# aptx4869lm/4DCapture-FPV

Hardware: AMD Instinct MI355X
Metric: frames/sec global-opt (fixed iters), 1024f clip/500k-pt scene; Chamfer GB/s (higher is better)
Workload: dtype f32; 1 GPU; BASELINE config 3: 1024-frame clip, 500000-pt scene, 500 contact verts, 500 Adam iterations (phase split 0.8), full loss; frames sharded over 1 GPU(s); frames=1024, scene_points=500000, contact_verts=500, iters=500, body_verts=10475, lbs_weights_per_vertex=4

## Files before the change

### 4dcapture-fpv_amd/capi.py

```python
from __future__ import annotations

import ctypes
import os
from ctypes import POINTER, c_char_p, c_double, c_float, c_int32, c_int64, c_void_p

import numpy as np

_HERE = os.path.dirname(os.path.abspath(__file__))
LIB_PATH = os.environ.get("FDCAP_LIB") or os.path.join(_HERE, "libfdcap_hip.so")

NUM_LOSSES = 8
XDIM = 78
PDIM = 75


class FdcapError(RuntimeError):
    pass


class ModelDesc(ctypes.Structure):
    _fields_ = [("num_verts", c_int32), ("v_template", POINTER(c_float)), ("shapedirs", POINTER(c_float)),
                ("num_shape", c_int32), ("posedirs", POINTER(c_float)), ("J_regressor", POINTER(c_float)),
                ("parents", POINTER(c_int32)), ("lbs_weights", POINTER(c_float)),
                ("hands_componentsl", POINTER(c_float)), ("hands_componentsr", POINTER(c_float)),
# ... 29 lines not shown
    "fdcap_debug_scene_hash": (c_int32, [c_void_p, c_void_p]),
    "fdcap_debug_scene_table": (c_int32, [c_void_p, c_int32, c_void_p, POINTER(c_int64)]),
    "fdcap_debug_kernel_forms": (c_int32, [c_void_p, c_int32, c_int32]),
    "fdcap_debug_pose_joint_sets": (c_int32, [c_void_p, c_void_p]),
    "fdcap_set_contact_ids": (c_int32, [c_void_p, c_void_p, c_int32]),
    "fdcap_chamfer_fwd": (c_int32, [c_void_p, c_void_p, c_void_p, c_int32, c_int32, c_int32, c_int64, c_void_p,
                                     c_void_p, c_void_p, c_void_p, c_void_p]),
    "fdcap_chamfer_bwd": (c_int32, [c_void_p, c_void_p, c_void_p, c_int32, c_int32, c_int32, c_int64, c_void_p,
                                     c_void_p, c_void_p, c_void_p]),
    "fdcap_chamfer_fwd_scene": (c_int32, [c_void_p, c_void_p, c_int32, c_int32, c_void_p, c_void_p, c_int32, c_void_p]),
    "fdcap_chamfer_bwd_scene": (c_int32, [c_void_p, c_void_p, c_int32, c_int32, c_void_p, c_void_p, c_void_p, c_void_p]),
    "fdcap_set_nn_kernel": (c_int32, [c_int32]),
    "fdcap_vposer_decode": (c_int32, [c_void_p, c_void_p, c_int32, c_int32, c_void_p, c_void_p, c_void_p]),
    "fdcap_vposer_decode_bwd": (c_int32, [c_void_p, c_void_p, c_int32, c_int32, c_void_p, c_void_p, c_void_p, c_void_p]),
    "fdcap_smplx_backward": (c_int32, [c_void_p] * 7 + [c_int32] + [c_void_p] * 9),
    "fdcap_body_forward": (c_int32, [c_void_p, c_void_p, c_int32, c_void_p, c_void_p, c_void_p]),
    "fdcap_world_mesh": (c_int32, [c_void_p, c_void_p, c_int32, c_void_p, c_void_p, c_void_p, c_void_p]),
    "fdcap_params_75_to_78": (c_int32, [c_void_p, c_int32, c_void_p, c_void_p]),
    "fdcap_params_78_to_75": (c_int32, [c_void_p, c_int32, c_void_p, c_void_p]),
    "fdcap_smplx_forward": (c_int32, [c_void_p, c_void_p, c_void_p, c_void_p, c_void_p, c_void_p, c_void_p, c_int32,
                                       c_void_p, c_void_p, c_void_p]),
    "fdcap_opt_create": (c_int32, [c_void_p, POINTER(OptConfig), c_void_p, c_void_p, c_void_p, c_void_p, c_void_p]),
    "fdcap_opt_create_clips": (c_int32, [c_void_p, POINTER(OptConfig), c_int32, c_void_p, c_void_p, c_void_p, c_void_p, c_void_p]),
    "fdcap_opt_create_clips_var": (c_int32, [c_void_p, POINTER(OptConfig), c_int32, POINTER(c_int32), c_void_p, c_void_p, c_void_p, c_void_p,
                                             c_void_p]),
    "fdcap_opt_set_inputs": (c_int32, [c_void_p, c_void_p, c_void_p, c_void_p, c_void_p, c_void_p]),
    "fdcap_opt_backward": (c_int32, [c_void_p, c_int32, c_int32, c_int32, c_void_p]),
    "fdcap_opt_step": (c_int32, [c_void_p, c_int32, c_int32, c_void_p]),
    "fdcap_opt_backward_and_step": (c_int32, [c_void_p, c_int32, c_int32, c_int32, c_void_p]),
    "fdcap_opt_sync": (c_int32, [c_void_p, c_void_p]),
    "fdcap_opt_run": (c_int32, [c_void_p, c_int32, c_int32, c_int32, c_int32, c_int32, c_void_p, c_int32, c_int32, c_void_p, c_void_p]),
    "fdcap_comm_unique_id": (c_int32, [c_void_p]),
    "fdcap_comm_create": (c_int32, [c_void_p, c_void_p, c_int32, c_int32]),
    "fdcap_comm_destroy": (c_int32, [c_void_p]),
    "fdcap_comm_last_error": (c_char_p, [c_void_p]),
    "fdcap_opt_halo_exchange": (c_int32, [c_void_p, c_void_p]),
    "fdcap_opt_exchange": (c_int32, [c_void_p, c_int32, c_int32, c_void_p]),
    "fdcap_opt_time_exchange": (c_int32, [c_void_p, c_int32, POINTER(c_float), POINTER(c_float), c_void_p]),
    "fdcap_comm_allreduce_f64": (c_int32, [c_void_p, c_void_p, c_int32, c_void_p]),
    "fdcap_opt_state_len": (c_int32, [c_void_p]),
    "fdcap_opt_export_state": (c_int32, [c_void_p, c_void_p, c_void_p]),
    "fdcap_opt_import_state": (c_int32, [c_void_p, c_void_p, c_void_p]),
    "fdcap_opt_check_finite": (c_int32, [c_void_p, c_void_p, c_void_p]),
    "fdcap_opt_set_loss_output": (c_int32, [c_void_p, c_void_p]),
    "fdcap_opt_detect_contact": (c_int32, [c_void_p, c_int32, c_void_p, c_void_p]),
    "fdcap_opt_backward_local2": (c_int32, [c_void_p, c_void_p, c_int32, c_void_p]),
    "fdcap_opt_step_x": (c_int32, [c_void_p, c_int32, c_void_p]),
    "fdcap_opt_set_dct": (c_int32, [c_void_p, c_void_p, c_int32, c_int32, c_void_p, c_void_p]),
    "fdcap_opt_dct_fit": (c_int32, [c_void_p, c_int32, c_int32, c_float, c_void_p, c_int32, c_void_p]),
    "fdcap_opt_backward_dct": (c_int32, [c_void_p, c_float, c_float, c_float, c_int32, c_void_p]),
    "fdcap_opt_set_dct_coef": (c_int32, [c_void_p, c_void_p, c_void_p]),
    "fdcap_opt_get_dct": (c_int32, [c_void_p, c_void_p, c_void_p]),
    "fdcap_opt_get_dct_state": (c_int32, [c_void_p, c_void_p, c_void_p, c_void_p]),
    "fdcap_opt_set_dct_state": (c_int32, [c_void_p, c_void_p, c_void_p, c_void_p]),
    "fdcap_opt_dct_windows": (c_int32, [c_void_p, POINTER(c_int32), POINTER(c_int32)]),
    "fdcap_frame_smoother": (c_int32, [c_void_p, c_void_p, c_int32, c_int32, c_float, c_float, c_float, c_float,
                                        c_void_p, c_int32, c_int32, c_void_p, c_void_p]),
    "fdcap_opt_set_keypoints": (c_int32, [c_void_p, c_void_p, c_void_p]),
    "fdcap_opt_backward_fit2d": (c_int32, [c_void_p, POINTER(Fit2dStage), c_int32, c_void_p]),
    "fdcap_opt_reset_adam": (c_int32, [c_void_p, c_void_p]),
    "fdcap_lbfgs_create": (c_int32, [c_int32, POINTER(LbfgsConfig), POINTER(c_void_p)]),
    "fdcap_lbfgs_destroy": (None, [c_void_p]),
    "fdcap_lbfgs_reset": (c_int32, [c_void_p, c_void_p]),
    "fdcap_lbfgs_advance": (c_int32, [c_void_p, c_void_p, c_int32, c_void_p, c_void_p, c_int32, c_void_p, c_void_p]),
    "fdcap_lbfgs_get_stats": (c_int32, [c_void_p, c_void_p, c_void_p, c_void_p, c_void_p]),
    "fdcap_lbfgs_finalize": (c_int32, [c_void_p, c_void_p, c_int32, c_void_p, c_void_p]),
    "fdcap_opt_fit2d_lbfgs": (c_int32, [c_void_p, POINTER(Fit2dStage), POINTER(LbfgsConfig), c_int32, POINTER(c_int32), c_void_p]),
    "fdcap_opt_fit2d_lbfgs_stats": (c_int32, [c_void_p, c_void_p, c_void_p, c_void_p, c_void_p]),
    "fdcap_opt_step_rows_and_pack": (c_int32, [c_void_p, c_int32, c_int32, c_void_p, c_void_p]),
    "fdcap_opt_unpack_and_step_scale": (c_int32, [c_void_p, c_int32, c_int32, c_void_p, c_int32, c_int32, c_void_p]),
    "fdcap_opt_forward_ahead": (c_int32, [c_void_p, c_int32, c_int32, c_int32, c_void_p]),
    "fdcap_exchange_len": (c_int32, []),
    "fdcap_opt_get_results": (c_int32, [c_void_p, c_void_p, c_void_p, c_void_p, c_void_p]),
    "fdcap_opt_destroy": (None, [c_void_p]),
    "fdcap_opt_forward_world": (c_int32, [c_void_p, c_void_p, c_void_p, c_void_p]),
    "fdcap_opt_get_contact": (c_int32, [c_void_p, c_void_p, c_void_p, c_void_p]),
    "fdcap_opt_get_grads": (c_int32, [c_void_p, c_void_p, c_void_p, c_void_p]),
    "fdcap_panel_gemm": (c_int32, [c_void_p, c_int32, c_int32, c_int32, c_void_p, c_int64, c_int64, c_int32, c_void_p, c_int32,
                                   c_void_p]),
    "fdcap_time_blend_gemm": (c_int32, [c_void_p, c_int32, c_int32, POINTER(c_float), c_void_p]),
    "fdcap_opt_nn_timing": (c_int32, [c_void_p, c_int32]),
    "fdcap_opt_nn_timing_read": (c_int32, [c_void_p, POINTER(c_float), POINTER(c_int32)]),
    "fdcap_debug_nn_query_order": (c_int32, [c_void_p, c_int32, c_void_p, c_int32]),
    "fdcap_debug_nn_query_sort": (c_int32, [c_void_p, c_void_p, c_int32, c_int32, c_int32, c_void_p, c_void_p, c_void_p]),
    "fdcap_opt_launch_timing": (c_int32, [c_void_p, c_int32]),
    "fdcap_opt_launch_timing_read": (c_int32, [c_void_p, c_void_p, c_void_p]),
    "fdcap_opt_time_chamfer": (c_int32, [c_void_p, c_int32, c_int32, POINTER(c_float), c_void_p]),
}

_lib = None


def load_library(path: str | None = None) -> ctypes.CDLL:
    global _lib
    if _lib is not None and path is None:
        return _lib
    p = path or LIB_PATH
    if not os.path.exists(p):
        raise FdcapError(f"{p} is missing: build it with `python -c 'import __graft_entry__ as g; g.build()'` "
                         "(hipcc --offload-arch=gfx950).  There is no CPU fallback.")
    lib = ctypes.CDLL(p)
    for name, (res, args) in SYMBOLS.items():
        fn = getattr(lib, name)
        fn.restype = res
        fn.argtypes = args
    info = lib.fdcap_build_info().decode()
    if "packed_fp32=off" not in info and os.environ.get("FDCAP_ALLOW_PK_F32") != "1":
        raise FdcapError(f"{p} was built with packed fp32 instructions ({info}): results are not reliable next to another kernel's "
                         "MFMAs on the same CU (NOTES.md section 6).  Rebuild with __graft_entry__.build(), or set "
                         "FDCAP_ALLOW_PK_F32=1 for an instrumentation variant.")
    if path is None:
        _lib = lib
    return lib


def count_packed_fp32(path: str | None = None) -> int:
    import re
    import shutil
    import subprocess
    import tempfile
    objdump = os.environ.get("LLVM_OBJDUMP", "/opt/rocm/lib/llvm/bin/llvm-objdump")
    if not os.path.exists(objdump):
        raise FdcapError(f"{objdump} not found (set LLVM_OBJDUMP)")
    with tempfile.TemporaryDirectory() as tmp:
        so = os.path.join(tmp, "lib.so")
        shutil.copy(path or LIB_PATH, so)
        subprocess.run([objdump, "--offloading", so], check=True, capture_output=True, cwd=tmp)
        objs = [f for f in os.listdir(tmp) if "amdgcn" in f]
        if not objs:
            raise FdcapError("no gfx950 code object found in the library")
        n = 0
        for f in objs:
            txt = subprocess.run([objdump, "-d", os.path.join(tmp, f)], check=True, capture_output=True, text=True).stdout
            n += len(re.findall(r"\bv_pk_(?:fma|mul|add)_f32\b", txt))
        return n


def check(code: int, what: str) -> None:
    if code == 0:
        return
    if code < 0:
        names = {-1: "FDCAP_E_ARG", -2: "FDCAP_E_STATE", -3: "FDCAP_E_NODEVICE", -4: "FDCAP_E_COMM (RCCL)"}
        raise FdcapError(f"{what}: {names.get(code, code)}")
    raise FdcapError(f"{what}: hipError_t {code}")


def _f32(a):
    return np.ascontiguousarray(a, dtype=np.float32)


def _fp(a):
    return a.ctypes.data_as(POINTER(c_float))


def dptr(t):
    if t is None:
        return None
    if not t.is_cuda:
        raise FdcapError("expected a device tensor (the HIP path has no host fallback)")
    if not t.is_contiguous():
        raise FdcapError("expected a contiguous tensor")
    return c_void_p(t.data_ptr())


def current_stream():
    import torch
# ... 58 lines not shown
```

### 4dcapture-fpv_amd/csrc/fdc_api_opt.h

```cpp
#pragma once

extern "C" {

void fdcap_opt_destroy(fdcap_ctx* c) {
    if (!c || !c->opt) return;
    OptState* o = c->opt;
    DevBuf<float>* fb[] = {&o->X0, &o->mask, &o->mX, &o->vX, &o->mCAM, &o->vCAM, &o->mS, &o->vS,
                           &o->H1, &o->H2, &o->O, &o->dO, &o->Opart, &o->dZpart, &o->Rm, &o->PF, &o->Jrest, &o->G, &o->A, &o->M,
                           &o->Jw, &o->Voff, &o->Vw, &o->dist, &o->pd, &o->dVoff, &o->dA, &o->dtransl_v, &o->dMv,
                           &o->dsv, &o->dPF, &o->dJw, &o->dX, &o->dCAM, &o->dscale_row, &o->loss_rows, &o->VoffF, &o->VwF, &o->dVF};
    for (auto* b : fb) b->release();
    o->dctD.release(); o->dctCoef.release(); o->dctM.release(); o->dctV.release(); o->adam_tab.release();
    o->clip_rows.release(); o->clip_span.release();
    o->idx.release(); o->pi.release(); o->seedpt.release(); o->kp2d.release(); o->floss.release();
    if (o->lbfgs) { fdcap_lbfgs_destroy(o->lbfgs); o->lbfgs = nullptr; }
    o->nnc_ids.release(); o->nnc_hdr.release(); o->nnc_anchor.release();
    for (hipEvent_t e : o->nn_ev) (void)hipEventDestroy(e);
    o->nn_ev.clear();
    for (hipEvent_t e : o->lt.ev) (void)hipEventDestroy(e);
    o->lt.ev.clear(); o->lt.what.clear(); o->lt.on = false; o->lt.used = 0;
    delete o;
    c->opt = nullptr;
}

static_assert(LROW == FDCAP_NUM_LOSSES, "a batch's per-clip loss slots are LROW apart on the device");
static_assert(CLIP_XDIM == XDIM && CLIP_NJW == NJW, "fdc_clips.h restates the two dimensions its weights divide by");
static_assert(POSE_NJ == NJ && POSE_NJW == NJW, "fdc_forms.h restates the two joint counts plan_pose_joints works with");

static LossWeights opt_phase_weights(const fdcap_opt_config& cf, bool phase2) {
    LossWeights lw;
    lw.rec = 1.f;
    lw.smooth = phase2 ? cf.phase2_smooth : cf.phase1_smooth;
    lw.contact = phase2 ? 0.f : cf.phase1_contact;
    lw.world = phase2 ? cf.phase2_world : 0.f;
    lw.dct = 0.f;
    lw.world_on = phase2;
    return lw;
}

static int opt_create_impl(fdcap_ctx* c, const fdcap_opt_config* cfg, int32_t n_clips, const int32_t* var_len, float* rows_x, float* rows_cam,
                           float* scale_d, float* dscale_d, double* losses_d) {
    SetupTrace tr("fdcap_opt_create");
    OptState* o = c->opt ? c->opt : new OptState();
    c->opt = o;
    o->cfg = *cfg;
    o->nclip = n_clips;
    o->clip_len = var_len ? 0 : cfg->n_total;
    o->ragged = var_len != nullptr;
    if (var_len) o->clip_lens.assign(var_len, var_len + n_clips);
    else o->clip_lens.assign((size_t)n_clips, cfg->n_total);
    o->clip_start = clip_starts(n_clips, o->clip_lens.data());
    if (n_clips > 1 && !var_len) o->cfg.n_total = o->cfg.n_local = n_clips * cfg->n_total;
    cfg = &o->cfg;
    o->cam_steps = 0;
    o->dz_pending = false;
    o->log_pending = false;
    o->seeded = false;
    o->dctT = o->dctC = o->dctW = 0;
    o->dct_grad = false;
    const int R = o->R = cfg->n_local + 4;
    o->contact_on = c->ns > 0 && c->nc > 0 && cfg->weight_contact != 0.f;
    const size_t nq = (size_t)R * std::max(c->nc, 1);
    o->sw = forms_read_env();
    { const char* e = getenv("FDCAP_POSE_TRIM"); o->sw.pose_trim = !(e && e[0] == '0'); }
    const int nq_all = (int)((size_t)cfg->n_local * c->nc);
    o->nsplit = o->contact_on ? nn_pick_nsplit(nq_all, (int)c->ns, o->sw.nn_seed && o->sw.nn_cull) : 1;
    o->nsplit_bf = o->contact_on ? nn_pick_nsplit(nq_all, (int)c->ns, false) : 1;
    int err = 0;
#define AL(buf, cnt) if (!err) { hipError_t e_ = (buf).ensure(cnt); if (e_ != hipSuccess) err = (int)e_; else e_ = hipMemset((buf).p, 0, (size_t)(cnt) * sizeof(*(buf).p)); }
    o->X.p = rows_x; o->CAM.p = rows_cam; o->scale.p = scale_d; o->dscale.p = dscale_d; o->losses.p = losses_d;
    o->pend.on = false;
    AL(o->X0, (size_t)R * XDIM) AL(o->mask, R)
    AL(o->mX, (size_t)R * XDIM) AL(o->vX, (size_t)R * XDIM) AL(o->mCAM, (size_t)R * 16) AL(o->vCAM, (size_t)R * 16)
    AL(o->mS, n_clips) AL(o->vS, n_clips)
    AL(o->H1, (size_t)R * 512) AL(o->H2, (size_t)R * 512) AL(o->O, (size_t)R * O_LD) AL(o->dO, (size_t)R * ODIM)
    AL(o->Opart, (size_t)4 * R * ODIM) AL(o->dZpart, (size_t)4 * R * VP_Z)
    AL(o->Rm, (size_t)R * RM_LD) AL(o->PF, (size_t)R * NPFX) AL(o->Jrest, (size_t)R * JR_LD) AL(o->G, (size_t)R * NJ * 12)
    AL(o->A, (size_t)R * NJ * 12) AL(o->M, (size_t)R * 12) AL(o->Jw, (size_t)R * NJW * 3)
    AL(o->dA, (size_t)R * NJ * 12) AL(o->dtransl_v, (size_t)R * 3) AL(o->dMv, (size_t)R * 12)
    AL(o->dsv, R) AL(o->dPF, (size_t)2 * R * NPFX)
    AL(o->dJw, (size_t)R * NJW * 3) AL(o->dX, (size_t)R * XDIM)
    AL(o->dCAM, (size_t)R * 16) AL(o->dscale_row, R) AL(o->loss_rows, (size_t)R * LROW)
    if (o->contact_on) {
        AL(o->Voff, nq * 3) AL(o->Vw, nq * 3) AL(o->dist, nq) AL(o->idx, nq) AL(o->dVoff, nq * 3) AL(o->seedpt, nq)
        AL(o->pd, (size_t)std::max(o->nsplit, o->nsplit_bf) * nq) AL(o->pi, (size_t)std::max(o->nsplit, o->nsplit_bf) * nq)
    }
#undef AL
    tr.mark("buffers");
    if (!err && o->contact_on) {
        hipError_t e_ = hipMemset(o->idx.p, 0xFF, nq * sizeof(int));
        if (e_ != hipSuccess) err = (int)e_;
    }
    if (!err && o->contact_on) {
        const int every = o->sw.nn_order;
        o->nn_order = NNOrder{};
        if (o->sw.nn_cache_slack > 0.f) {
            const size_t ng = ((size_t)nq_all + 31) / 32, ng4 = ng * 4;
            hipError_t e_ = o->nnc_ids.ensure(ng4 * NN_CACHE_CAP);
            if (e_ == hipSuccess) e_ = o->nnc_hdr.ensure(ng4 + 3 * ng);
            if (e_ == hipSuccess) e_ = o->nnc_anchor.ensure((size_t)4 * nq_all);
            if (e_ == hipSuccess && every > 0) e_ = o->nnq_buf.ensure(nn_query_order_ints(nq_all));
            if (e_ == hipSuccess) e_ = hipMemset(o->nnc_hdr.p, 0xFF, ng4 * sizeof(int));
            if (e_ == hipSuccess) e_ = hipMemset(o->nnc_hdr.p + ng4, 0, 3 * ng * sizeof(int));
            if (e_ == hipSuccess) e_ = hipMemset(o->nnc_anchor.p, 0, (size_t)4 * nq_all * sizeof(float4));
            if (e_ != hipSuccess) err = (int)e_;
            if (every > 0) { o->nn_order.on = true; o->nn_order.every = every; o->nn_order.qbuf = o->nnq_buf.p; }
        }
    }
    if (!err) {
        const std::vector<float> s((size_t)n_clips, cfg->scale_init);
        hipError_t e_ = hipMemcpy(o->scale.p, s.data(), s.size() * sizeof(float), hipMemcpyHostToDevice);
        if (e_ != hipSuccess) err = (int)e_;
    }
    if (!err && o->ragged) {
        std::vector<ClipRow> rows = clip_rows_build(n_clips, var_len, opt_phase_weights(*cfg, false), cfg->weight_loss_rec, cfg->weight_contact, c->nc);
        const std::vector<ClipRow> rows2 = clip_rows_build(n_clips, var_len, opt_phase_weights(*cfg, true), cfg->weight_loss_rec, cfg->weight_contact, c->nc);
        rows.insert(rows.end(), rows2.begin(), rows2.end());
        std::vector<int> span((size_t)2 * n_clips);
        for (int k = 0; k < n_clips; ++k) { span[(size_t)2 * k] = o->clip_start[(size_t)k]; span[(size_t)2 * k + 1] = var_len[k]; }
        hipError_t e_ = rows.size() == (size_t)2 * R ? o->clip_rows.upload(rows.data(), rows.size()) : hipErrorInvalidValue;
        if (e_ == hipSuccess) e_ = o->clip_span.upload(span.data(), span.size());
        if (e_ != hipSuccess) err = (int)e_;
    }
    tr.mark("search state");
    if (err) { fdcap_opt_destroy(c); return err; }
    return FDCAP_OK;
}

int fdcap_opt_create_clips(fdcap_ctx* c, const fdcap_opt_config* cfg, int32_t n_clips, float* rows_x, float* rows_cam, float* scale_d,
                           float* dscale_d, double* losses_d) {
    if (!c || !cfg || !rows_x || !rows_cam || !scale_d || !dscale_d || !losses_d || cfg->n_local <= 0 || cfg->n_total < cfg->n_local || cfg->frame0 < 0 ||
        cfg->frame0 + cfg->n_local > cfg->n_total || n_clips < 1)
        return FDCAP_E_ARG;
    if (n_clips > 1 && (cfg->frame0 != 0 || cfg->n_local != cfg->n_total || (int64_t)n_clips * cfg->n_total > (1 << 24)))
        return FDCAP_E_ARG;
    return opt_create_impl(c, cfg, n_clips, nullptr, rows_x, rows_cam, scale_d, dscale_d, losses_d);
}

int fdcap_opt_create_clips_var(fdcap_ctx* c, const fdcap_opt_config* cfg, int32_t n_clips, const int32_t* clip_len, float* rows_x, float* rows_cam,
                               float* scale_d, float* dscale_d, double* losses_d) {
    if (!c || !cfg || !rows_x || !rows_cam || !scale_d || !dscale_d || !losses_d || cfg->frame0 != 0 || cfg->n_local != cfg->n_total ||
        !clip_lengths_ok(n_clips, clip_len, cfg->n_total, (int64_t)1 << 24))
        return FDCAP_E_ARG;
    if (clip_lengths_equal(n_clips, clip_len)) {
        fdcap_opt_config one = *cfg;
        one.n_total = one.n_local = clip_len[0];
        return fdcap_opt_create_clips(c, &one, n_clips, rows_x, rows_cam, scale_d, dscale_d, losses_d);
// ... 49 lines not shown
    const bool timed = o->nn_timing && o->nn_ev_used + 2 <= (int)o->nn_ev.size();
    if (timed) HIP_TRY(hipEventRecord(o->nn_ev[o->nn_ev_used], st));
    {
        TraceRange tr_("fdcap:chamfer_nn(K14)");
        HIP_TRY(nn_search(o->Vw.p + off, nq, c->nn_target(o->sw.nn_cull), o->dist.p + 2 * nc, o->idx.p + 2 * nc, o->pd.p, o->pi.p,
                          o->nsplit, st, o->sw.nn_seed ? o->idx.p + 2 * nc : nullptr, !o->seeded, o->seedpt.p + 2 * nc, &o->nnpt_valid,
                          &cache, &o->nn_order));
    }
    if (timed) { HIP_TRY(hipEventRecord(o->nn_ev[o->nn_ev_used + 1], st)); o->nn_ev_used += 2; }
    lt_mark(o, FDCAP_LT_CHAMFER_NN, st);
    o->seeded = true;
    return 0;
}

static int opt_backward_impl(fdcap_ctx* c, const LossWeights& lw, int32_t log_terms, hipStream_t st, int fuse_ii = -1, int fuse_P = 0) {
    OptState* o = c->opt;
    const fdcap_opt_config& cf = o->cfg;
    const int nl = cf.n_local, nc = c->nc, N = o->clip_len, rpc = o->rows_per_clip(), kn = o->kclip_n();
    const ClipRow* ctab = nullptr;
    if (o->ragged) {
        const auto same = [&lw](const LossWeights& t) {
            return t.rec == lw.rec && t.smooth == lw.smooth && t.contact == lw.contact && t.world == lw.world && t.dct == lw.dct && t.world_on == lw.world_on;
        };
        if (same(opt_phase_weights(cf, false))) ctab = o->ctab(false);
        else if (same(opt_phase_weights(cf, true))) ctab = o->ctab(true);
        else return FDCAP_E_STATE;
    }
    const int* const cspan = o->cspan();
    const bool dct_on = lw.dct != 0.f && o->dctW > 0;
    PoseModel pm = c->pose_model();
    TraceRange tr_(fuse_ii >= 0 ? "fdcap:backward_and_step" : "fdcap:backward");
    if (o->log_pending) {
        hipLaunchKernelGGL(loss_rows_reduce_kernel, dim3(o->nclip), dim3(256), 0, st, o->loss_rows.p, 2, rpc, o->log_mask, o->log_assign, o->log_dst,
                           o->dscale_row.p, o->dscale.p, cspan);
        o->log_pending = false;
    }
    double* const losses = log_terms ? o->losses.p : nullptr;
    const bool rows_log = losses && o->dctW == 0;
    if (losses && !rows_log) HIP_TRY(hipMemsetAsync(losses, 0, (size_t)o->nclip * FDCAP_NUM_LOSSES * sizeof(double), st));
    int row_lo, row_hi;
    opt_row_range(o, 1, &row_lo, &row_hi);
    const bool ahead = o->ahead, blend_done = o->ahead && o->ahead_blend;
    const bool contact_grad = o->contact_on && lw.contact != 0.f;
    const bool contact_fwd = o->contact_on && (contact_grad || log_terms);
    o->lt.phase = contact_grad ? 0 : 1;
    const bool contact_state = contact_fwd || (dct_on || o->dctW > 0);
    const bool need_world = lw.world_on || dct_on || o->dctW > 0 || log_terms != 0 || ahead || cf.n_local != cf.n_total;
    const PoseJoints pj = plan_pose_joints(c->h_parents.data(), c->h_depth.data(), contact_fwd ? c->contact.ja_hi : 0, contact_state, need_world,
                                           o->sw.pose_trim && o->dctW == 0);
    if (contact_grad && (pj.jr != NJ || pj.jn < c->contact.ja_hi)) return FDCAP_E_STATE;
    int e = ahead ? opt_pose_forward_rest(c, row_lo, row_hi, st) : opt_pose_forward(c, row_lo, row_hi, st, contact_state, &pj);
    o->ahead = false;
    if (e) return e;
    if (contact_fwd) { e = opt_contact_forward(c, st, blend_done); if (e) return e; }
    const ClipWeights cw = clip_weights(std::max(N, 1), lw, cf.weight_loss_rec, cf.weight_contact, nc);
    const float w_rec = cw.w_rec, w_sm = cw.w_sm, w_ws = cw.w_ws;
    const bool fuse_pl = (!losses || rows_log) && !(o->dctW > 0 && dct_on);
    ParamLossIn pli = {};
    if (fuse_pl) pli = ParamLossIn{o->X0.p, o->mask.p, o->Jw.p, cf.frame0, N, w_rec, w_sm, w_ws, lw.world_on ? 1 : 0,
                                   rows_log ? o->loss_rows.p : nullptr};
    else if (ctab) return FDCAP_E_STATE;
    else
        hipLaunchKernelGGL(param_loss_kernel, dim3(nl), dim3(128), 0, st, o->X.p, o->X0.p, o->mask.p, o->Jw.p, 2, cf.frame0, N,
                           w_rec, w_sm, w_ws, lw.world_on ? 1 : 0, o->dX.p, o->dJw.p, losses, kn);
    if (o->dctW > 0 && (dct_on || log_terms))
        hipLaunchKernelGGL(dct_joint_grad_kernel, dim3((nl * 69 + 255) / 256), dim3(256), 0, st, o->Jw.p, 2, cf.frame0, nl, o->dctT,
                           o->dctC, o->dctW, o->dctD.p, o->dctCoef.p, dct_on ? lw.dct / (69.f * (float)o->dctW) : 0.f,
                           lw.world_on ? 1 : 0, o->dJw.p, losses ? losses + 7 : nullptr);
    o->dct_grad = dct_on;
    bool dpf_split = false;
    int dA_rows = NJ;
    if (contact_grad) {
        ContactGradIn cg;
        cg.Vw = o->Vw.p; cg.dist = o->dist.p; cg.idx = o->idx.p; cg.scene = c->scene.p;
        cg.nnpt = o->nnpt_valid ? o->seedpt.p : nullptr;
        cg.coef = cw.coef;
        cg.loss_rows = losses ? o->loss_rows.p : nullptr;
        const SkinModel smc = c->contact.model();
        const int nnz = c->contact.nnz;
        const bool aligned16 = (((size_t)o->Vw.p | (size_t)o->Voff.p | (size_t)o->dVoff.p | (size_t)o->A.p) & 15) == 0;
        const SkinBwdPlan pl = plan_contact_skin_bwd(nl, nc, nnz, smc.K, smc.vpack != nullptr, smc.csc_v16 != nullptr, aligned16, smc.wf_tab != nullptr,
                                                     o->sw.skin_vec);
        if (pl.ja_rows) dA_rows = c->contact.ja_hi;
        const dim3 grid(pl.grid), block(pl.block);
#define FDC_SKC(KERNEL) hipLaunchKernelGGL(KERNEL, grid, block, pl.lds, st, smc, nc, nnz, o->X.p, o->Voff.p, o->A.p, o->M.p, o->scale.p, 2, o->dVoff.p, \
                                           o->dA.p, o->dtransl_v.p, o->dMv.p, o->dsv.p, cg, kn, ctab)
        switch (pl.form) {
        case F_SKIN_BWD_VEC:
            note_form(form_name(pl.form));
            if (pl.G == 1) FDC_SKC(skin_bwd_vec_kernel<1>); else if (pl.G == 2) FDC_SKC(skin_bwd_vec_kernel<2>); else FDC_SKC(skin_bwd_vec_kernel<3>);
            break;
        case F_SKIN_BWD_SMALL: case F_SKIN_BWD_SMALL_K:
            note_form(form_name(pl.form));
            if (pl.vpt == 2 && pl.kc == 8) FDC_SKC((skin_bwd_small_kernel<2, 8>));
            else if (pl.vpt == 2) FDC_SKC((skin_bwd_small_kernel<2, 24>));
            else if (pl.kc == 16) FDC_SKC((skin_bwd_small_kernel<4, 16>));
            else FDC_SKC((skin_bwd_small_kernel<4, 24>));
            break;
        default:
            { int es = skin_bwd_any<true>(c->ws_skin, st, nl, smc, nc, o->X.p, o->Voff.p, o->A.p, o->M.p, o->scale.p, 2,
                                          (const float*)nullptr, o->dVoff.p, o->dA.p, (float*)nullptr, o->dtransl_v.p, o->dMv.p, o->dsv.p, cg, kn, ctab);
              if (es) return es; }
        }
#undef FDC_SKC
        lt_mark(o, FDCAP_LT_SKIN_BWD, st);
        HIP_TRY(blend_backward(c->contact, o->dVoff.p + (size_t)2 * nc * 3, nl, o->dPF.p + 2 * NPFX, (size_t)o->R * NPFX, c->ws_kpart, st, &dpf_split));
        lt_mark(o, FDCAP_LT_BLEND_BWD, st);
    } else if (contact_fwd && losses) {
        if (fuse_pl && rows_log) { pli.cdist = o->dist.p; pli.cnc = nc; }
        else hipLaunchKernelGGL(contact_loss_rows_kernel, dim3(nl), dim3(256), 0, st, o->dist.p, nc, 2, o->loss_rows.p);
    }
    const bool joint_grad = lw.world_on || dct_on;
    hipLaunchKernelGGL(pose_bwd_kernel, dim3(nl), dim3(64 * POSE_NW), 0, st, pm, o->X.p, o->O.p, o->CAM.p, o->scale.p, 2, o->Rm.p,
                       o->Jrest.p, o->G.p, contact_grad ? o->dA.p : nullptr, contact_grad ? o->dPF.p : nullptr,
                       joint_grad ? o->dJw.p : nullptr, contact_grad ? o->dMv.p : nullptr, contact_grad ? o->dsv.p : nullptr,
                       contact_grad ? o->dPF.p + NPF : nullptr, NPFX, contact_grad ? o->dtransl_v.p : nullptr, o->dX.p, o->dO.p,
                       o->dCAM.p, o->dscale_row.p, pli, (contact_grad && dpf_split) ? (const float*)(o->dPF.p + (size_t)o->R * NPFX) : (const float*)nullptr,
                       dA_rows, kn, ctab, pj.jn, pj.jr, pj.nlev);
    o->pj_bwd = pj;
    lt_mark(o, FDCAP_LT_POSE_BWD, st);
    const unsigned log_mask = (rows_log ? 0x17u : 0u) | (contact_fwd ? 0x8u : 0u);
    bool log_in_tail = false;
    {
        ScaleTail tail;
        if (fuse_ii >= 0) {
            const StepPlan sp = opt_step_plan(o, fuse_ii, fuse_P, false, true);
            tail.dscale_row = o->dscale_row.p; tail.row0 = 2;
            if (sp.step_scale) {
                tail.block = 0; tail.sc = sp.sc; tail.dscale = o->dscale.p; tail.n = rpc;
                tail.zero_grad = fuse_ii >= fuse_P ? 1 : 0;
            }
            if (log_terms == 2 && rows_log) {
                tail.block = 0; tail.lg = LogReduceIn{o->loss_rows.p, losses, log_mask, 1, rpc};
                log_in_tail = true;
            }
        }
        int eb = opt_vposer_backward(c, false, st, tail);
        if (eb) return eb;
        if (fuse_ii >= 0) { o->pend.on = true; o->pend.ii = fuse_ii; o->pend.P = fuse_P; }
    }
    if (log_terms && !log_in_tail) {
        if (log_terms == 2 && rows_log) {
            o->log_pending = true; o->log_mask = log_mask; o->log_assign = 1; o->log_dst = losses;
        } else
            hipLaunchKernelGGL(loss_rows_reduce_kernel, dim3(o->nclip), dim3(256), 0, st, o->loss_rows.p, 2, rpc, log_mask, rows_log ? 1 : 0, losses,
                               o->dscale_row.p, o->dscale.p, cspan);
    }
    return (int)hipGetLastError();
}

int fdcap_opt_set_loss_output(fdcap_ctx* c, double* losses_d) {
    if (!c || !c->opt || !losses_d) return FDCAP_E_ARG;
    c->opt->log_pending = false;
    c->opt->log_dst = nullptr;
    c->opt->losses.p = losses_d;
    return FDCAP_OK;
}

int fdcap_opt_forward_ahead(fdcap_ctx* c, int32_t ii, int32_t P, int32_t log_terms, void* stream) {
    if (!c || !c->opt || c->opt->nclip > 1) return FDCAP_E_STATE;
    { int es_ = opt_sync(c, (hipStream_t)stream); if (es_) return es_; }
    OptState* o = c->opt;
    hipStream_t st = (hipStream_t)stream;
    const int nl = o->cfg.n_local, nc = c->nc;
    int e = opt_pose_forward(c, 2, 2 + nl, st);
    if (e) return e;
// ... 78 lines not shown
```

### 4dcapture-fpv_amd/csrc/fdc_api_run.h

```cpp
#pragma once

extern "C" {

int fdcap_opt_detect_contact(fdcap_ctx* c, int32_t n_left, float* weight_left, void* stream) {
    if (opt_is_batch(c)) return FDCAP_E_STATE;
    if (!c || !c->opt || !weight_left || n_left <= 0 || n_left > c->nc) return FDCAP_E_ARG;
    OptState* o = c->opt;
    if (!o->contact_on) return FDCAP_E_STATE;
    hipStream_t st = (hipStream_t)stream;
    const int nl = o->cfg.n_local, nc = c->nc;
    int row_lo, row_hi;
    opt_row_range(o, 1, &row_lo, &row_hi);
    int e = opt_pose_forward(c, row_lo, row_hi, st);
    if (e) return e;
    e = opt_contact_forward(c, st);
    if (e) return e;
    hipLaunchKernelGGL(detect_contact_kernel, dim3(nl), dim3(256), 0, st, o->dist.p, c->contact_perm.p, nc, n_left, 2, weight_left);
    return (int)hipGetLastError();
}

int fdcap_opt_backward_local2(fdcap_ctx* c, const float* contact_weight, int32_t n_left, void* stream) {
    if (opt_is_batch(c)) return FDCAP_E_STATE;
    if (!c || !c->opt || !contact_weight || n_left <= 0 || n_left >= c->nc) return FDCAP_E_ARG;
    { int es_ = opt_sync(c, (hipStream_t)stream); if (es_) return es_; }
// ... 200 lines not shown
    int e = comm_buffers(c);
    if (e) return e;
    hipEvent_t ev[4];
    for (auto& x : ev) HIP_TRY(hipEventCreate(&x));
    const int big = 1 << 30;
    for (int k = 0; k < 8 && !e; ++k) e = fdcap_opt_exchange(c, k, big, stream);
    if (!e) e = (int)hipEventRecord(ev[0], st);
    for (int k = 0; k < iters && !e; ++k) e = fdcap_opt_exchange(c, 8 + k, big, stream);
    if (!e) e = (int)hipEventRecord(ev[1], st);
    if (!e) e = (int)hipEventRecord(ev[2], st);
    for (int k = 0; k < iters && !e; ++k) {
        const ncclResult_t r = rccl().AllGather(c->xch_send.p, c->xch_all.p, XCH_LEN, ncclFloat, c->comm.comm, st);
        if (r != ncclSuccess) e = comm_fail(c, r, "ncclAllGather");
    }
    if (!e) e = (int)hipEventRecord(ev[3], st);
    if (!e) e = (int)hipEventSynchronize(ev[3]);
    float a = 0.f, b = 0.f;
    if (!e) e = (int)hipEventElapsedTime(&a, ev[0], ev[1]);
    if (!e) e = (int)hipEventElapsedTime(&b, ev[2], ev[3]);
    for (auto& x : ev) (void)hipEventDestroy(x);
    *us_exchange = a * 1e3f / iters;
    *us_allgather = b * 1e3f / iters;
    return e;
}

int fdcap_opt_run(fdcap_ctx* c, int32_t ii0, int32_t ii1, int32_t num_iter, int32_t P, int32_t log_every, double* hist_d,
                  int32_t hist_rows, int32_t flags, int32_t* n_logged, void* stream) {
    if (n_logged) *n_logged = 0;
    if (!c || !c->opt) return FDCAP_E_STATE;
    if (ii0 < 0 || ii1 < ii0 || ii1 > num_iter || log_every < 0) return FDCAP_E_ARG;
    OptState* o = c->opt;
    const bool sharded = (flags & 2) != 0 || !opt_whole_clips(o);
    if (sharded && (!c->comm.comm || o->nclip > 1)) return FDCAP_E_STATE;
    const size_t hist_row = (size_t)o->nclip * FDCAP_NUM_LOSSES;
    double* const keep = o->losses.p;
    int k = 0, e = 0;
    for (int ii = ii0; ii < ii1 && !e; ++ii) {
        const bool do_log = log_every > 0 && (ii % log_every == 0 || ii == num_iter - 1);
        if (do_log) {
            if (!hist_d || k >= hist_rows) { e = FDCAP_E_ARG; break; }
            e = fdcap_opt_set_loss_output(c, hist_d + (size_t)k * hist_row);
            if (e) break;
            ++k;
        }
        const int lt = do_log ? 2 : 0;
        if (sharded) {
            e = fdcap_opt_backward(c, ii, P, lt, stream);
            if (!e) e = fdcap_opt_exchange(c, ii, P, stream);
        } else if (!(flags & 1) && ii + 1 < num_iter) {
            e = fdcap_opt_backward_and_step(c, ii, P, lt, stream);
        } else {
            e = fdcap_opt_backward(c, ii, P, lt, stream);
            if (!e) e = fdcap_opt_step(c, ii, P, stream);
        }
    }
    if (k) {
        const int e2 = fdcap_opt_set_loss_output(c, keep);
        if (!e) e = e2;
    }
    if (n_logged) *n_logged = k;
    return e;
}

int fdcap_comm_allreduce_f64(fdcap_ctx* c, double* buf_d, int32_t n, void* stream) {
    if (!c || !buf_d || n <= 0) return FDCAP_E_ARG;
    if (!c->comm.comm) return FDCAP_E_STATE;
    const ncclResult_t r = rccl().AllReduce(buf_d, buf_d, (size_t)n, ncclDouble, ncclSum, c->comm.comm, (hipStream_t)stream);
    if (r != ncclSuccess) return comm_fail(c, r, "ncclAllReduce");
    return FDCAP_OK;
}

int fdcap_opt_get_contact(fdcap_ctx* c, float* dist, int32_t* idx, void* stream) {
    if (!c || !c->opt) return FDCAP_E_STATE;
    OptState* o = c->opt;
    if (!o->contact_on) return FDCAP_E_STATE;
    hipStream_t st = (hipStream_t)stream;
    const size_t n = (size_t)o->cfg.n_local * c->nc;
    const int nl = o->cfg.n_local, nc = c->nc;
    if (dist) hipLaunchKernelGGL(unpermute_kernel<float>, dim3((n + 255) / 256), dim3(256), 0, st, o->dist.p + 2 * nc,
                                 c->contact_perm.p, nl, nc, 1, dist);
    if (idx) hipLaunchKernelGGL(unpermute_kernel<int>, dim3((n + 255) / 256), dim3(256), 0, st, o->idx.p + 2 * nc,
                                c->contact_perm.p, nl, nc, 1, idx);
    return (int)hipGetLastError();
}

int fdcap_opt_get_grads(fdcap_ctx* c, float* dx, float* dcam, void* stream) {
    if (!c || !c->opt) return FDCAP_E_STATE;
    { int es_ = opt_sync(c, (hipStream_t)stream); if (es_) return es_; }
    OptState* o = c->opt;
    hipStream_t st = (hipStream_t)stream;
    const int nl = o->cfg.n_local;
    if (o->dz_pending) {
        hipLaunchKernelGGL(vposer_fold_dz_kernel, dim3((nl * VP_Z + 255) / 256), dim3(256), 0, st, o->dZpart.p, (size_t)o->R * VP_Z, 2, nl, o->dX.p);
        o->dz_pending = false;
    }
    if (dx) HIP_TRY(hipMemcpyAsync(dx, o->dX.p + 2 * XDIM, (size_t)nl * XDIM * sizeof(float), hipMemcpyDeviceToDevice, st));
    if (dcam) HIP_TRY(hipMemcpyAsync(dcam, o->dCAM.p + 2 * 16, (size_t)nl * 16 * sizeof(float), hipMemcpyDeviceToDevice, st));
    return FDCAP_OK;
}

int fdcap_panel_gemm(const float* A, int32_t lda, int32_t M, int32_t K, const float* B_h, int64_t sk, int64_t sn, int32_t N, float* C,
                     int32_t ldc, void* stream) {
    if (!A || !B_h || !C || M <= 0 || K <= 0 || N <= 0 || lda < K || ldc < N) return FDCAP_E_ARG;
    hipStream_t st = (hipStream_t)stream;
    {
        if (forms_read_env().gemm_split3 && panel_gemm3_fits(K)) {
            std::vector<unsigned> p3;
            std::vector<float> sc;
            PanelB3 B3;
            PnF::pack(B_h, (long)sk, (long)sn, K, N, p3, sc, &B3.ntile, &B3.nst);
            DevBuf<unsigned> d3;
            DevBuf<float> ds;
            HIP_TRY(d3.upload(p3.data(), p3.size()));
            HIP_TRY(ds.upload(sc.data(), sc.size()));
            B3.f = (const uint4*)d3.p; B3.isc = ds.p;
            hipError_t e = panel_gemm3(A, lda, M, K, B3, C, ldc, N, st);
            hipError_t e2 = hipStreamSynchronize(st);
            d3.release(); ds.release();
            return (int)(e != hipSuccess ? e : e2);
        }
    }
    std::vector<float> pf;
    PanelB B;
    panel_pack(B_h, (long)sk, (long)sn, K, N, pf, &B.ntile, &B.nss);
    DevBuf<float> d;
    HIP_TRY(d.upload(pf.data(), pf.size()));
    B.f = (const float4*)d.p;
    hipError_t e = panel_gemm(A, lda, M, K, B, C, ldc, N, st);
    hipError_t e2 = hipStreamSynchronize(st);
    d.release();
    return (int)(e != hipSuccess ? e : e2);
}

int fdcap_opt_nn_timing(fdcap_ctx* c, int32_t max_launches) {
    if (!c || !c->opt || max_launches < 0) return FDCAP_E_ARG;
    OptState* o = c->opt;
    o->nn_timing = max_launches > 0;
    o->nn_ev_used = 0;
    while ((int)o->nn_ev.size() < 2 * max_launches) {
        hipEvent_t e;
        HIP_TRY(hipEventCreate(&e));
        o->nn_ev.push_back(e);
    }
    return FDCAP_OK;
}
int fdcap_opt_nn_timing_read(fdcap_ctx* c, float* mean_ms, int32_t* launches) {
    if (!c || !c->opt || !mean_ms || !launches) return FDCAP_E_ARG;
    OptState* o = c->opt;
    double sum = 0.0;
    for (int i = 0; i + 1 < o->nn_ev_used; i += 2) {
        HIP_TRY(hipEventSynchronize(o->nn_ev[i + 1]));
        float t = 0.f;
        HIP_TRY(hipEventElapsedTime(&t, o->nn_ev[i], o->nn_ev[i + 1]));
        sum += t;
    }
    *launches = o->nn_ev_used / 2;
    *mean_ms = *launches ? (float)(sum / *launches) : 0.f;
    return FDCAP_OK;
}

int fdcap_opt_launch_timing(fdcap_ctx* c, int32_t max_events) {
    if (!c || !c->opt || max_events < 0) return FDCAP_E_ARG;
    OptState::LaunchTimes& t = c->opt->lt;
    t.on = max_events > 0;
    t.used = 0;
    while ((int)t.ev.size() < max_events) {
// ... 95 lines not shown
```

### 4dcapture-fpv_amd/csrc/fdc_chamfer.h

```cpp
#pragma once
#include <hip/hip_runtime.h>
#include <stdlib.h>

#include <atomic>

#include "fdc_forms.h"
#include "fdc_math.h"

namespace fdc {

constexpr int NN_TILE = 1024;

struct NNTarget {
    const float4* pts;
    int n;
    const float4* bounds;
    const float4* sbounds;
    const float4* qbounds;
    const int* inv_perm;
    const uint4* frags;
    const float4* centers;
};

__device__ __forceinline__ float nn_exact_d2(float qx, float qy, float qz, float px, float py, float pz) {
    float dx = qx - px, dy = qy - py, dz = qz - pz;
    return __fmaf_rn(dz, dz, __fmaf_rn(dy, dy, __fmul_rn(dx, dx)));
}
__device__ __forceinline__ bool nn_better(float d, int i, float bd, int bi) {
    return d < bd || (d == bd && i < bi);
}

__device__ __forceinline__ void nn_block_map(int b, int nsplit, int* qb, int* split) {
    const int xcd = b & 7, slot = b >> 3;
    *split = slot % nsplit;
    *qb = (slot / nsplit) * 8 + xcd;
}

template <int QPT>
__global__ __launch_bounds__(256) void nn_direct_kernel(const float* __restrict__ q, int nq, NNTarget T, int nsplit,
                                                        float* __restrict__ pd, int* __restrict__ pi) {
    __shared__ float4 tile[NN_TILE];
    const int tid = threadIdx.x;
    int split, qb;
    nn_block_map(blockIdx.x, nsplit, &qb, &split);
    if (qb * (256 * QPT) >= nq) return;
    const int per = nn_split_len(T.n, nsplit);
    const int t_begin = min(T.n, split * per);
    const int t_end = min(T.n, t_begin + per);
    float qx[QPT], qy[QPT], qz[QPT], best[QPT];
    int bi[QPT];
#pragma unroll
    for (int u = 0; u < QPT; ++u) {
        int qi = qb * (256 * QPT) + u * 256 + tid;
        bool ok = qi < nq;
        qx[u] = ok ? q[3 * (size_t)qi] : 0.f;
        qy[u] = ok ? q[3 * (size_t)qi + 1] : 0.f;
        qz[u] = ok ? q[3 * (size_t)qi + 2] : 0.f;
        best[u] = INFINITY;
        bi[u] = -1;
    }
    for (int base = t_begin; base < t_end; base += NN_TILE) {
        const int cnt = min(NN_TILE, t_end - base);
        for (int j = tid; j < cnt; j += 256) tile[j] = T.pts[base + j];
        __syncthreads();
#pragma unroll 4
        for (int j = 0; j < cnt; ++j) {
            const float4 p = tile[j];
            const int gi = __float_as_int(p.w);
#pragma unroll
            for (int u = 0; u < QPT; ++u) {
                float d = nn_exact_d2(qx[u], qy[u], qz[u], p.x, p.y, p.z);
                if (nn_better(d, gi, best[u], bi[u])) { best[u] = d; bi[u] = gi; }
            }
        }
        __syncthreads();
    }
#pragma unroll
    for (int u = 0; u < QPT; ++u) {
        int qi = qb * (256 * QPT) + u * 256 + tid;
        if (qi < nq) {
            pd[(size_t)split * nq + qi] = best[u];
            pi[(size_t)split * nq + qi] = bi[u];
        }
    }
}

#ifndef FDC_MF_K1
#define FDC_MF_K1 1e-4f
#endif
#ifndef FDC_MF_K2
#define FDC_MF_K2 8e-6f
#endif
constexpr float MF_K1 = FDC_MF_K1, MF_K2 = FDC_MF_K2;

#ifdef FDC_NN_TIMELINE
__device__ unsigned long long g_nn_timeline[16384 * 8];
#endif
#ifdef FDC_NN_STATS
__device__ unsigned long long g_nn_hist[96];
__device__ unsigned long long g_nn_stats[8];
#define FDC_STAT(i, v) st_cnt[i] += (v)
#else
#define FDC_STAT(i, v)
#endif

typedef __bf16 bf16x8 __attribute__((ext_vector_type(8)));
typedef float f32x16_t __attribute__((ext_vector_type(16)));

__device__ __forceinline__ unsigned f2bf(float f) {
    __bf16 h = (__bf16)f;
    return (unsigned)__builtin_bit_cast(unsigned short, h);
}
__device__ __forceinline__ float bf2f(unsigned h) { return __uint_as_float(h << 16); }
// ... 201 lines not shown
                    FDC_STAT(1, lane == 0);
#pragma unroll
                    for (int r = 0; r < 16; ++r) {
                        if (acc[r] < thr[n]) {
                            FDC_STAT(2, 1);
                            const int row = (r & 3) + 8 * (r >> 2) + 4 * half;
                            const float4 p = sP[buf][tile * 32 + row];
                            const int gi = __float_as_int(p.w);
                            const float d = nn_exact_d2(qx[n], qy[n], qz[n], p.x, p.y, p.z);
                            if (base + tile * 32 + row < t_end && nn_better(d, gi, own_d[n], own_i[n])) {
                                own_d[n] = d;
                                own_i[n] = gi;
                                thr[n] = mf_thr(d, X[n], X2[n]);
                            }
                        }
                    }
                    const float sb = fminf(own_d[n], __shfl_xor(own_d[n], 32, 64));
                    if (qidx[n] < nq) thr[n] = mf_thr(sb, X[n], X2[n]);
                }
            }
        }
        if (more) stage_write(buf ^ 1, nxt);
        __syncthreads();
        buf ^= 1;
    }
#ifdef FDC_NN_STATS
    for (int i = 0; i < 8; ++i) atomicAdd(&g_nn_stats[i], (unsigned long long)st_cnt[i]);
#endif
#pragma unroll
    for (int n = 0; n < NQ; ++n) {
        float od = __shfl_xor(own_d[n], 32, 64);
        int oi = __shfl_xor(own_i[n], 32, 64);
        if (oi >= 0 && (own_i[n] < 0 || nn_better(od, oi, own_d[n], own_i[n]))) { own_d[n] = od; own_i[n] = oi; }
        if (half == 0 && qidx[n] < nq) {
            pd[(size_t)split * nq + qidx[n]] = own_d[n];
            pi[(size_t)split * nq + qidx[n]] = own_i[n];
        }
    }
}


#ifndef FDC_ST4_MAXLIST
#define FDC_ST4_MAXLIST 768
#endif
#ifndef FDC_ST4_MAXCELL
#define FDC_ST4_MAXCELL 256
#endif
constexpr int ST4_MAXLIST = FDC_ST4_MAXLIST;
constexpr int ST4_MAXCELL = FDC_ST4_MAXCELL;
#ifndef FDC_ST4_PF
#define FDC_ST4_PF 2
#endif
#ifndef FDC_AS_MULT
#define FDC_AS_MULT 4.f
#endif
#ifndef FDC_AS_MAX
#define FDC_AS_MAX 3.f
#endif
#ifndef FDC_AS_NEAR
#define FDC_AS_NEAR 0.8f
#endif
#ifndef FDC_ST4_OCC
#define FDC_ST4_OCC 8
#endif
#ifndef FDC_ST4_OCC2
#define FDC_ST4_OCC2 3
#endif
constexpr int ST4_PF = FDC_ST4_PF;
constexpr int ST4_SUPER = 16;
constexpr int ST4_QCAP = 8;

#ifndef FDC_NN_CACHE_CAP
#define FDC_NN_CACHE_CAP 128
#endif
constexpr int NN_CACHE_CAP = FDC_NN_CACHE_CAP;
static_assert(NN_CACHE_CAP == 64 || NN_CACHE_CAP == 128, "one or two ids per lane");
struct NNCache {
    unsigned short* ids;
    int* hdr;
    float4* anchor;
    float slack;
    int order_mode = 0;
    const int* perm = nullptr;
};

template <int NQ, int WPG, int WPB = 4>
__global__ __launch_bounds__(64 * WPB, NQ == 1 ? FDC_ST4_OCC : FDC_ST4_OCC2) void nn_stream4_kernel(const float* __restrict__ q, int nq, NNTarget T,
                                                         const int* __restrict__ seed, float4* __restrict__ seedpt,
                                                         float* __restrict__ dist, int* __restrict__ idx, NNCache cache) {
    __shared__ unsigned short slist[WPB][ST4_MAXLIST];
    __shared__ unsigned short clist[WPB][ST4_MAXCELL];
    __shared__ float4 sbox[WPB][64][2];
    __shared__ float s_d[WPB][32 * NQ];
    __shared__ int s_i[WPB][32 * NQ];
    __shared__ float4 s_p[WPB][32 * NQ];
    __shared__ int s_q[WPB][32 * NQ];
    static_assert(WPG == 1 || WPG == 2 || WPG == 4, "waves per query group");
    static_assert(WPB % WPG == 0 && WPB <= 4, "a group's waves share a workgroup");
    constexpr int GPW = WPB / WPG;
    constexpr int CPS = ST4_SUPER / WPG;
    const int tid = threadIdx.x, wave = tid >> 6, lane = tid & 63, half = lane >> 5, col = lane & 31;
    const int sub = wave % WPG, gslot = wave / WPG;
    const int ngroups = (nq + 32 * NQ - 1) / (32 * NQ);
    const int nwg = (ngroups + GPW - 1) / GPW;
#ifdef FDC_NN_TIMELINE
    const unsigned long long tl_t0 = wall_clock64();
    unsigned long long tl_p[4] = {0, 0, 0, 0};
#define TL_STAMP(k) tl_p[k] = wall_clock64()
#else
#define TL_STAMP(k)
#endif
    const int wg = (cache.order_mode >= 2 && (int)blockIdx.x < nwg) ? cache.hdr[(3 + cache.order_mode) * ((nq + 31) / 32) + (int)blockIdx.x] : (int)blockIdx.x;
    const int group = wg * GPW + gslot;
    const bool idle = wg >= nwg || group >= ngroups;
    const int wq0 = idle ? nq : group * (32 * NQ);
    const int nchunk = (T.n + MF_CH - 1) / MF_CH;
    const int myn = idle ? 0 : (nchunk - sub + WPG - 1) / WPG;
#ifdef FDC_NN_STATS
    unsigned st_cnt[8] = {0, 0, 0, 0, 0, 0, 0, 0};
#endif
    const bool caching = cache.hdr != nullptr && !idle;
    const int cidx = group * WPG + sub;
    float lqx[NQ], lqy[NQ], lqz[NQ];
    int lsj[NQ];
    float4 lsp[NQ];
    const int* const perm = NQ == 1 && WPB == 1 ? cache.perm : nullptr;
#pragma unroll
    for (int n = 0; n < NQ; ++n) {
        size_t qc = (size_t)min(wq0 + n * 32 + col, nq - 1);
        if (perm) {
            qc = (size_t)perm[qc];
            if (half == 0) s_q[wave][n * 32 + col] = (int)qc;
        }
        lqx[n] = q[3 * qc]; lqy[n] = q[3 * qc + 1]; lqz[n] = q[3 * qc + 2];
        lsj[n] = seed[qc];
        lsp[n] = seedpt[qc];
    }
    int hv_pre = -1;
    unsigned id_pre = 0;
    float4 anc_pre[NQ];
#pragma unroll
    for (int n = 0; n < NQ; ++n) anc_pre[n] = make_float4(0.f, 0.f, 0.f, -1.f);
    if (caching) {
        hv_pre = cache.hdr[cidx];
        id_pre = NN_CACHE_CAP == 64 ? (unsigned)cache.ids[(size_t)cidx * NN_CACHE_CAP + lane]
                                    : ((const unsigned*)cache.ids)[(size_t)cidx * (NN_CACHE_CAP / 2) + lane];
#pragma unroll
        for (int n = 0; n < NQ; ++n) anc_pre[n] = cache.anchor[(size_t)sub * nq + min(wq0 + n * 32 + col, nq - 1)];
    }
#if defined(__HIP_DEVICE_COMPILE__)
#pragma unroll
    for (int n = 0; n < NQ; ++n)
        asm volatile("" : "+v"(lqx[n]), "+v"(lqy[n]), "+v"(lqz[n]), "+v"(lsj[n]), "+v"(lsp[n].x), "+v"(lsp[n].y), "+v"(lsp[n].z), "+v"(lsp[n].w),
                          "+v"(anc_pre[n].x), "+v"(anc_pre[n].y), "+v"(anc_pre[n].z), "+v"(anc_pre[n].w), "+v"(hv_pre), "+v"(id_pre));
#endif
    float qx[NQ], qy[NQ], qz[NQ], own_d[NQ], sb[NQ];
    int own_i[NQ], qidx[NQ];
    float4 own_p[NQ];
    bool all_seeded = true;
#pragma unroll
    for (int n = 0; n < NQ; ++n) {
        qidx[n] = wq0 + n * 32 + col;
        const bool ok = qidx[n] < nq;
        qx[n] = ok ? lqx[n] : 0.f;
        qy[n] = ok ? lqy[n] : 0.f;
        qz[n] = ok ? lqz[n] : 0.f;
        own_d[n] = INFINITY;
        own_i[n] = -1;
        own_p[n] = make_float4(0.f, 0.f, 0.f, __int_as_float(-1));
        const int sj = ok ? lsj[n] : -1;
        const float4 p = ok ? lsp[n] : make_float4(0.f, 0.f, 0.f, 0.f);
        if (ok) {
            if (sj >= 0 && sj < T.n) {
                own_p[n] = p;
                own_d[n] = nn_exact_d2(qx[n], qy[n], qz[n], p.x, p.y, p.z);
                own_i[n] = sj;
            } else {
                all_seeded = false;
            }
        }
        sb[n] = ok ? own_d[n] * 1.00002f + 1e-9f : -INFINITY;
    }
    float rq[NQ];
    bool finite = true;
#pragma unroll
    for (int n = 0; n < NQ; ++n) {
        rq[n] = 0.f;
        if (qidx[n] < nq) {
            rq[n] = __builtin_amdgcn_sqrtf(sb[n]) * 1.00001f + 1e-6f;
            finite &= rq[n] < INFINITY;
        }
    }
    const bool cull = __all(all_seeded && finite);
    TL_STAMP(0);
    auto min_rows01 = [](float v) {
        v = fminf(v, dpp_move<0xB1>(v)); v = fminf(v, dpp_move<0x4E>(v)); v = fminf(v, dpp_move<0x141>(v)); v = fminf(v, dpp_move<0x140>(v));
        return fminf(__int_as_float(__builtin_amdgcn_readlane(__float_as_int(v), 0)), __int_as_float(__builtin_amdgcn_readlane(__float_as_int(v), 16)));
    };
    auto max_rows01 = [](float v) {
        v = fmaxf(v, dpp_move<0xB1>(v)); v = fmaxf(v, dpp_move<0x4E>(v)); v = fmaxf(v, dpp_move<0x141>(v)); v = fmaxf(v, dpp_move<0x140>(v));
        return fmaxf(__int_as_float(__builtin_amdgcn_readlane(__float_as_int(v), 0)), __int_as_float(__builtin_amdgcn_readlane(__float_as_int(v), 16)));
    };

    int n_kept = -1;
    bool inflate = false;
    int slk = __builtin_amdgcn_readfirstlane(__float_as_int(cache.slack));
    if (cull && caching) {
        const int hv = __builtin_amdgcn_readfirstlane(hv_pre);
        bool ok = true;
        float dmax = 0.f;
#pragma unroll
        for (int n = 0; n < NQ; ++n)
            if (qidx[n] < nq) {
                const float4 a = anc_pre[n];
                const float ex = qx[n] - a.x, ey = qy[n] - a.y, ez = qz[n] - a.z;
                const float dl = __builtin_amdgcn_sqrtf(ez * ez + (ey * ey + ex * ex)) * 1.00001f + 1e-7f;
                ok &= rq[n] + dl <= a.w;
                dmax = fmaxf(dmax, dl);
            }
        if (hv >= 0 && __all(ok)) {
            n_kept = hv & 255;
            if (lane == 0) cache.hdr[cidx] = hv + 256;
        } else {
            dmax = max_rows01(dmax);
            dmax = fmaxf(dmax, __shfl_xor(dmax, 32, 64));
            const float age = hv >= 0 ? (float)max(hv >> 8, 1) : 1.f;
            const float speed = dmax / age;
            slk = __builtin_amdgcn_readfirstlane(__float_as_int(fminf(fmaxf(FDC_AS_MULT * speed, cache.slack), FDC_AS_MAX * cache.slack)));
            float smin = __int_as_float(slk);
#pragma unroll
            for (int n = 0; n < NQ; ++n)
                if (qidx[n] < nq && rq[n] > FDC_AS_NEAR) smin = fminf(smin, fmaxf(cache.slack, __int_as_float(slk) * (FDC_AS_NEAR / rq[n])));
            smin = -max_rows01(-smin);
            smin = fminf(smin, __shfl_xor(smin, 32, 64));
            inflate = 3.f * speed <= smin;
        }
    }
    auto slack_of = [&](float r) -> float {
        const float sw = __int_as_float(slk);
        return r <= FDC_AS_NEAR ? sw : fmaxf(cache.slack, sw * (FDC_AS_NEAR / r));
    };
    float sbT[NQ];
    float glx = INFINITY, gly = INFINITY, glz = INFINITY, ghx = -INFINITY, ghy = -INFINITY, ghz = -INFINITY;
    float scx = 0.f, scy = 0.f, scz = 0.f, sR2 = 0.f;
    if (cull && n_kept < 0) {
        float rT[NQ];
#pragma unroll
        for (int n = 0; n < NQ; ++n) {
            rT[n] = inflate ? rq[n] + slack_of(rq[n]) : rq[n];
            sbT[n] = (qidx[n] < nq) ? (inflate ? rT[n] * rT[n] * 1.00002f : sb[n]) : -INFINITY;
        }
#pragma unroll
        for (int n = 0; n < NQ; ++n)
            if (qidx[n] < nq) {
                const float r = rT[n];
                glx = fminf(glx, qx[n] - r); gly = fminf(gly, qy[n] - r); glz = fminf(glz, qz[n] - r);
                ghx = fmaxf(ghx, qx[n] + r); ghy = fmaxf(ghy, qy[n] + r); ghz = fmaxf(ghz, qz[n] + r);
            }
        glx = min_rows01(glx); gly = min_rows01(gly); glz = min_rows01(glz);
        ghx = max_rows01(ghx); ghy = max_rows01(ghy); ghz = max_rows01(ghz);
        scx = 0.5f * (glx + ghx); scy = 0.5f * (gly + ghy); scz = 0.5f * (glz + ghz);
        float sR = 0.f;
#pragma unroll
        for (int n = 0; n < NQ; ++n)
            if (qidx[n] < nq) {
                const float ex = qx[n] - scx, ey = qy[n] - scy, ez = qz[n] - scz;
                sR = fmaxf(sR, (__builtin_amdgcn_sqrtf(ex * ex + ey * ey + ez * ez) + rT[n]) * 1.00001f + 1e-6f);
            }
        sR = max_rows01(sR);
        sR2 = sR * sR * 1.00001f;
    } else {
#pragma unroll
        for (int n = 0; n < NQ; ++n) sbT[n] = sb[n];
    }
    auto overlaps = [&](float4 lo, float4 hi) -> bool {
        return !((lo.x > ghx) | (hi.x < glx) | (lo.y > ghy) | (hi.y < gly) | (lo.z > ghz) | (hi.z < glz)) & (box_d2(lo, hi, scx, scy, scz) <= sR2);
    };
// ... 240 lines not shown
                            unsigned hi = 0;
#pragma unroll
                            for (int r = 15; r >= 9; --r) hi = __builtin_amdgcn_alignbit(hi, __float_as_uint(acc[r] - th), 31);
                            mask |= hi << 9;
                        }
                        if constexpr (NQ == 1) {
                            mask &= (seed_tile == (base >> 5) + tile) ? seed_keep : ~0u;
                        } else {
                            const int spos = __float_as_int(own_p[n].w);
                            const bool mine = (spos >> 5) == (base >> 5) + tile && ((spos >> 2) & 1) == half;
                            if (mine) mask &= ~(1u << ((spos & 3) + 4 * ((spos >> 3) & 3)));
                        }
                        if (!__any(mask != 0)) continue;
                        if constexpr (NQ == 1) {
                            while (mask) {
                                const int r = __ffs(mask) - 1;
                                mask &= mask - 1;
                                const int pos = base + tile * 32 + (r & 3) + 8 * (r >> 2) + 4 * half;
                                if (pos < T.n) {
                                    FDC_STAT(2, 1);
                                    if (cq_n < ST4_QCAP) { cq[cq_n * 64 + lane] = (unsigned)pos; ++cq_n; }
                                    else {
                                        const float4 p = T.pts[pos];
                                        const int gi = __float_as_int(p.w);
                                        const float d = nn_exact_d2(qx[n], qy[n], qz[n], p.x, p.y, p.z);
                                        if (nn_better(d, gi, own_d[n], own_i[n])) {
                                            own_d[n] = d; own_i[n] = gi;
                                            own_p[n] = make_float4(p.x, p.y, p.z, __int_as_float(pos));
                                            seed_refresh();
                                        }
                                    }
                                }
                            }
                            continue;
                        }
                        while (mask) {
                            const int r = __ffs(mask) - 1;
                            mask &= mask - 1;
                            const int pos = base + tile * 32 + (r & 3) + 8 * (r >> 2) + 4 * half;
                            if (pos < T.n && pos != __float_as_int(own_p[n].w)) {
                                FDC_STAT(2, 1);
                                const float4 p = T.pts[pos];
                                const int gi = __float_as_int(p.w);
                                const float d = nn_exact_d2(qx[n], qy[n], qz[n], p.x, p.y, p.z);
                                if (nn_better(d, gi, own_d[n], own_i[n])) {
                                    own_d[n] = d; own_i[n] = gi;
                                    own_p[n] = make_float4(p.x, p.y, p.z, __int_as_float(pos));
                                }
                            }
                        }
                        const float sbest = fminf(own_d[n], __shfl_xor(own_d[n], 32, 64));
                        if (qidx[n] < nq) thr[n] = fminf(thr[n], sbest + c2[n]);
                    }
                }
            }
            ch = ch_next;
            qd = id_next & 3;
            fo = fo_next;
        }
    }
    if constexpr (NQ == 1) {
        for (int k0 = 0; __any(k0 < cq_n); k0 += 4) {
            float4 p[4];
            int ps[4];
#pragma unroll
            for (int k = 0; k < 4; ++k) {
                ps[k] = (k0 + k < cq_n) ? (int)cq[(k0 + k) * 64 + lane] : 0;
                p[k] = T.pts[ps[k]];
            }
#pragma unroll
            for (int k = 0; k < 4; ++k)
                if (k0 + k < cq_n) {
                    const int gi = __float_as_int(p[k].w);
                    const float d = nn_exact_d2(qx[0], qy[0], qz[0], p[k].x, p[k].y, p[k].z);
                    if (nn_better(d, gi, own_d[0], own_i[0])) {
                        own_d[0] = d; own_i[0] = gi;
                        own_p[0] = make_float4(p[k].x, p[k].y, p[k].z, __int_as_float(ps[k]));
                    }
                }
        }
    }
    TL_STAMP(3);
    if (cache.order_mode != 0 && lane == 0 && !idle) cache.hdr[4 * ((nq + 31) / 32) + (int)blockIdx.x] = nsurv;
#pragma unroll
    for (int n = 0; n < NQ; ++n) {
        const float od = __shfl_xor(own_d[n], 32, 64);
        const int oi = __shfl_xor(own_i[n], 32, 64);
        float4 op;
        op.x = __shfl_xor(own_p[n].x, 32, 64); op.y = __shfl_xor(own_p[n].y, 32, 64);
        op.z = __shfl_xor(own_p[n].z, 32, 64); op.w = __shfl_xor(own_p[n].w, 32, 64);
        if (oi >= 0 && (own_i[n] < 0 || nn_better(od, oi, own_d[n], own_i[n]))) { own_d[n] = od; own_i[n] = oi; own_p[n] = op; }
        if (half == 0) { s_d[wave][n * 32 + col] = own_d[n]; s_i[wave][n * 32 + col] = own_i[n]; s_p[wave][n * 32 + col] = own_p[n]; }
    }
    __syncthreads();
#ifdef FDC_NN_STATS
    {
        unsigned mx = st_cnt[2];
        for (int off = 32; off > 0; off >>= 1) mx = max(mx, (unsigned)__shfl_xor((int)mx, off, 64));
        if (lane == 0 && !idle) {
            atomicAdd(&g_nn_hist[32 + (st_cnt[1] > 0 ? 32 - __clz(st_cnt[1]) : 0)], 1ull);
            atomicAdd(&g_nn_hist[64 + (mx > 0 ? 32 - __clz(mx) : 0)], 1ull);
        }
    }
    for (int i = 0; i < 8; ++i) atomicAdd(&g_nn_stats[i], (unsigned long long)st_cnt[i]);
#endif
#ifdef FDC_NN_TIMELINE
    if (tid == 0 && blockIdx.x < 16384) {
        unsigned xcc; asm volatile("s_getreg_b32 %0, hwreg(HW_REG_XCC_ID)" : "=s"(xcc));
        unsigned long long* tl = g_nn_timeline + (size_t)blockIdx.x * 8;
        tl[0] = tl_t0; tl[1] = wall_clock64(); tl[2] = xcc & 15; tl[3] = tl_p[0]; tl[4] = tl_p[1]; tl[5] = tl_p[2]; tl[6] = tl_p[3]; tl[7] = (unsigned long long)tl_nsurv;
    }
#endif
    if (tid < GPW * 32 * NQ) {
        const int g = tid / (32 * NQ), e = tid % (32 * NQ);
        const int qo = (wg * GPW + g) * (32 * NQ) + e;
        if (wg < nwg && qo < nq) {
            int bw = g * WPG;
            float bd = s_d[bw][e];
            int bi = s_i[bw][e];
#pragma unroll
            for (int w = 1; w < WPG; ++w) {
                const float d = s_d[g * WPG + w][e];
                const int i = s_i[g * WPG + w][e];
                if (i >= 0 && (bi < 0 || nn_better(d, i, bd, bi))) { bd = d; bi = i; bw = g * WPG + w; }
            }
            const int qd = perm ? s_q[g][e] : qo;
            dist[qd] = bd;
            idx[qd] = bi;
            seedpt[qd] = s_p[bw][e];
        }
    }
}

__global__ __launch_bounds__(256) void nn_seed_kernel(const float* __restrict__ q, int nq, NNTarget T, int* __restrict__ seed,
                                                      float4* __restrict__ seedpt) {
    const int qi = blockIdx.x * 256 + threadIdx.x;
    if (qi >= nq) return;
    const int old = seed[qi];
    if (old >= 0 && old < T.n) {
        const int pos = T.inv_perm ? T.inv_perm[old] : old;
        const float4 pt = T.pts[pos];
        seedpt[qi] = make_float4(pt.x, pt.y, pt.z, __int_as_float(pos));
        return;
    }
    const float x = q[3 * (size_t)qi], y = q[3 * (size_t)qi + 1], z = q[3 * (size_t)qi + 2];
    const int nchunk = (T.n + MF_CH - 1) / MF_CH;
    float bb = INFINITY;
    int bc = -1;
    int p0, p1;
    if (T.sbounds) {
        const int nsuper = (nchunk + ST4_SUPER - 1) / ST4_SUPER;
        for (int s = 0; s < nsuper; ++s) {
            const float ds = box_d2(T.sbounds[2 * s], T.sbounds[2 * s + 1], x, y, z);
            if (!(ds < bb)) continue;
            for (int c = s * ST4_SUPER; c < min(nchunk, (s + 1) * ST4_SUPER); ++c) {
                const float d = box_d2(T.bounds[2 * c], T.bounds[2 * c + 1], x, y, z);
                if (d < bb) { bb = d; bc = c; }
            }
        }
    } else {
        for (int c = 0; c < nchunk; ++c) {
            const float d = box_d2(T.bounds[2 * c], T.bounds[2 * c + 1], x, y, z);
            if (d < bb) { bb = d; bc = c; }
        }
    }
    if (bc < 0) return;
    float bd = INFINITY;
    int bi = -1;
    float4 bp = make_float4(0.f, 0.f, 0.f, __int_as_float(-1));
    auto scan = [&](int c) {
        p0 = c * MF_CH;
        p1 = min(T.n, p0 + MF_CH);
        for (int p = p0; p < p1; ++p) {
            const float4 pt = T.pts[p];
            const float d = nn_exact_d2(x, y, z, pt.x, pt.y, pt.z);
            if (d < bd) { bd = d; bi = __float_as_int(pt.w); bp = make_float4(pt.x, pt.y, pt.z, __int_as_float(p)); }
        }
    };
    scan(bc);
    if (T.centers) {
        float bm = INFINITY;
        int bc2 = -1;
        auto centre = [&](int c) {
            const float4 cc = T.centers[c];
            const float dx = x - cc.x, dy = y - cc.y, dz = z - cc.z;
            const float m = __builtin_amdgcn_sqrtf(fmaf(dz, dz, fmaf(dy, dy, dx * dx))) + cc.w;
            if (m < bm) { bm = m; bc2 = c; }
        };
        if (T.sbounds) {
            const int nsuper = (nchunk + ST4_SUPER - 1) / ST4_SUPER;
            for (int sb = 0; sb < nsuper; ++sb) {
                if (!(box_d2(T.sbounds[2 * sb], T.sbounds[2 * sb + 1], x, y, z) < bm * bm)) continue;
                for (int c = sb * ST4_SUPER; c < min(nchunk, (sb + 1) * ST4_SUPER); ++c) centre(c);
            }
        } else
            for (int c = 0; c < nchunk; ++c) centre(c);
        if (bc2 >= 0 && bc2 != bc && bm * bm < bd) scan(bc2);
    }
    seed[qi] = bi;
    seedpt[qi] = bp;
}

__global__ void nn_combine_kernel(const float* __restrict__ pd, const int* __restrict__ pi, int nsplit, int nq,
                                  float* __restrict__ dist, int* __restrict__ idx) {
    int qi = blockIdx.x * blockDim.x + threadIdx.x;
    if (qi >= nq) return;
    float best = INFINITY;
    int bi = -1;
    for (int s = 0; s < nsplit; ++s) {
        float d = pd[(size_t)s * nq + qi];
        int j = pi[(size_t)s * nq + qi];
        if (j >= 0 && (bi < 0 || nn_better(d, j, best, bi))) { best = d; bi = j; }
    }
    dist[qi] = best;
    idx[qi] = bi;
}

__global__ void pack_points_kernel(const float* __restrict__ xyz, int n, float4* __restrict__ out) {
    int i = blockIdx.x * blockDim.x + threadIdx.x;
    if (i >= n) return;
    out[i] = make_float4(xyz[3 * (size_t)i], xyz[3 * (size_t)i + 1], xyz[3 * (size_t)i + 2], __int_as_float(i));
}

__global__ void nn_grad_kernel(const float* __restrict__ q, const float4* __restrict__ tgt, const float* __restrict__ g,
                               const int* __restrict__ idx, int nq, float* __restrict__ gq) {
    int qi = blockIdx.x * blockDim.x + threadIdx.x;
    if (qi >= nq) return;
    int j = idx[qi];
    float gg = 2.f * g[qi];
    float4 p = j >= 0 ? tgt[j] : make_float4(0, 0, 0, 0);
    gq[3 * (size_t)qi] = j >= 0 ? gg * (q[3 * (size_t)qi] - p.x) : 0.f;
    gq[3 * (size_t)qi + 1] = j >= 0 ? gg * (q[3 * (size_t)qi + 1] - p.y) : 0.f;
    gq[3 * (size_t)qi + 2] = j >= 0 ? gg * (q[3 * (size_t)qi + 2] - p.z) : 0.f;
}

inline std::atomic<int>& nn_mode_ref() {
    static std::atomic<int> mode{0};
    return mode;
}

__global__ __launch_bounds__(1024) void nn_order_kernel(const int* __restrict__ work, int n, const int* __restrict__ prev,
                                                        int* __restrict__ order) {
    __shared__ int cnt[16][256], base[256];
    const int tid = threadIdx.x, w = tid >> 6;
    for (int e = tid; e < 16 * 256; e += 1024) (&cnt[0][0])[e] = 0;
    __syncthreads();
    for (int i = tid; i < n; i += 1024) atomicAdd(&cnt[w][255 - min(max(work[i], 0), 255)], 1);
    __syncthreads();
    if (tid < 256) {
        int run = 0;
        for (int k = 0; k < 16; ++k) { const int t = cnt[k][tid]; cnt[k][tid] = run; run += t; }
        base[tid] = run;
    }
    __syncthreads();
    if (tid < 64) {
        const int a = base[4 * tid], b = base[4 * tid + 1], c = base[4 * tid + 2], d = base[4 * tid + 3];
        int s = a + b + c + d, incl = s;
        for (int off = 1; off < 64; off <<= 1) { const int t = __shfl_up(incl, off, 64); if (tid >= off) incl += t; }
        const int ex = incl - s;
        base[4 * tid] = ex; base[4 * tid + 1] = ex + a; base[4 * tid + 2] = ex + a + b; base[4 * tid + 3] = ex + a + b + c;
    }
    __syncthreads();
    for (int i = tid; i < n; i += 1024) {
        const int k = 255 - min(max(work[i], 0), 255);
        order[base[k] + atomicAdd(&cnt[w][k], 1)] = prev ? prev[i] : i;
    }
}
struct NNOrder {
    bool on = false;
    int sorted_groups = 0;
    int cur = 0;
    int age = 0;
    int every = 32;
    int* qbuf = nullptr;
    int perm_n = 0;
    int perm_mode = 0;
};
static inline size_t nn_query_order_ints(int nq);
static inline hipError_t nn_query_order(const float4* seedpt, int nq, int* qbuf, int* hdr, int groups, hipStream_t st);

static inline hipError_t nn_search(const float* q, int nq, const NNTarget& T, float* dist, int* idx, float* pd, int* pi,
                                   int nsplit, hipStream_t st, const int* seed = nullptr, bool seed_missing = false,
                                   float4* seedpt = nullptr, bool* seedpt_written = nullptr, const NNCache* cache = nullptr,
                                   NNOrder* ord = nullptr) {
    if (seedpt_written) *seedpt_written = false;
    if (nq <= 0) return hipSuccess;
    const NNPlan pl = plan_nn_search(nq, T.n, seed != nullptr && T.bounds != nullptr, T.frags != nullptr, seedpt != nullptr && seed == idx, nsplit,
                                     nn_mode_ref(), proc_switches());
    const dim3 grid(pl.grid), block(pl.block);
    note_form(form_name(pl.form));
    if (pl.wpg) {
        if (seed_missing)
            hipLaunchKernelGGL(nn_seed_kernel, dim3((nq + 255) / 256), dim3(256), 0, st, q, nq, T, idx, seedpt);
        if (seedpt_written) *seedpt_written = true;
        {
            const int groups = pl.groups, wpg = pl.wpg;
            NNCache nc = cache ? *cache : NNCache{nullptr, nullptr, nullptr, 0.f};
            const bool ordered = ord != nullptr && ord->on && nc.hdr != nullptr && ord->every > 0 && wpg == 1;
            nc.order_mode = !ordered ? 0 : (ord->sorted_groups == groups ? 2 + ord->cur : 1);
            const bool qorder = ordered && ord->qbuf != nullptr && ord->perm_mode != 1;
            nc.perm = qorder && ord->perm_n == nq ? ord->qbuf : nullptr;
            if (wpg == 4) hipLaunchKernelGGL((nn_stream4_kernel<1, 4>), grid, block, 0, st, q, nq, T, seed, seedpt, dist, idx, nc);
            else if (wpg == 2) hipLaunchKernelGGL((nn_stream4_kernel<1, 2>), grid, block, 0, st, q, nq, T, seed, seedpt, dist, idx, nc);
            else hipLaunchKernelGGL((nn_stream4_kernel<1, 1, 1>), grid, block, 0, st, q, nq, T, seed, seedpt, dist, idx, nc);
            const bool resort = ordered && (ord->sorted_groups != groups || ++ord->age >= ord->every);
            if (qorder && ord->perm_mode == 0 && (ord->perm_n != nq || seed_missing || (resort && ord->sorted_groups == groups))) {
                const hipError_t e = nn_query_order(seedpt, nq, ord->qbuf, nc.hdr, groups, st);
                if (e != hipSuccess) return e;
                ord->perm_n = nq;
                ord->sorted_groups = 0;
                ord->age = 0;
            } else if (resort) {
                const bool had = nc.order_mode >= 2;
                const int nxt = had ? 1 - ord->cur : 0;
                hipLaunchKernelGGL(nn_order_kernel, dim3(1), dim3(1024), 0, st, (const int*)(nc.hdr + 4 * groups), groups,
                                   had ? (const int*)(nc.hdr + (5 + ord->cur) * groups) : (const int*)nullptr, nc.hdr + (5 + nxt) * groups);
                ord->cur = nxt;
                ord->sorted_groups = groups;
                ord->age = 0;
            }
        }
        return hipGetLastError();
    }
    if (pl.form == F_NN_MFMA && pl.nq_blocks == 2) hipLaunchKernelGGL((nn_mfma_kernel<2>), grid, block, 0, st, q, nq, T, nsplit, seed, pd, pi);
    else if (pl.form == F_NN_MFMA) hipLaunchKernelGGL((nn_mfma_kernel<4>), grid, block, 0, st, q, nq, T, nsplit, seed, pd, pi);
    else hipLaunchKernelGGL((nn_direct_kernel<2>), grid, block, 0, st, q, nq, T, nsplit, pd, pi);
    hipLaunchKernelGGL(nn_combine_kernel, dim3((nq + 255) / 256), dim3(256), 0, st, pd, pi, nsplit, nq, dist, idx);
    return hipGetLastError();
}

}
```

### 4dcapture-fpv_amd/csrc/fdc_forms.h

```cpp
#pragma once
#include <stddef.h>
#include <stdlib.h>

#include <algorithm>

#if defined(__HIPCC__)
#define FDC_FORMS_HD __host__ __device__
#else
#define FDC_FORMS_HD
#endif

namespace fdc {

struct FormSwitches {
    int clip_fwd_rows = 336;
    int clip_kgrad_rows = 257;
    int pn_rb2 = 1;
    int pn_nw = 0;
    bool pn_ksw = true;
    bool gemm_split3 = true;
    int nn_stream = -2;
    bool nn_seed = true, nn_cull = true;
    int nn_order = 32;
    float nn_cache_slack = 0.03f;
    bool skin_vec = true;
    bool fuse_skin = true;
    bool pose_trim = true;
};
inline FormSwitches forms_read_env() {
    FormSwitches s;
    const auto off = [](const char* name) { const char* e = getenv(name); return e && e[0] == '0'; };
    if (const char* e = getenv("FDCAP_CLIP_FORMS_MIN_ROWS")) s.clip_fwd_rows = s.clip_kgrad_rows = std::max(32, atoi(e));
    if (const char* e = getenv("FDCAP_PN_RB2")) s.pn_rb2 = atoi(e);
    if (const char* e = getenv("FDCAP_PN_NW")) s.pn_nw = atoi(e);
    s.pn_ksw = !off("FDCAP_PN_KSW");
    s.gemm_split3 = !off("FDCAP_GEMM_SPLIT3");
    if (const char* e = getenv("FDCAP_NN_STREAM")) s.nn_stream = atoi(e);
    s.nn_seed = !off("FDCAP_NN_SEED");
    s.nn_cull = !off("FDCAP_NN_CULL");
    if (const char* e = getenv("FDCAP_NN_ORDER")) s.nn_order = atoi(e);
    if (const char* e = getenv("FDCAP_NN_CACHE_SLACK")) s.nn_cache_slack = (float)atof(e);
    s.skin_vec = !off("FDCAP_SKIN_VEC");
    s.fuse_skin = !off("FDCAP_FUSE_SKIN");
    return s;
}
inline const FormSwitches& proc_switches() { static const FormSwitches s = forms_read_env(); return s; }

enum Form {
    F_NONE = 0,
    F_PANEL3, F_PANEL3_RB2, F_PANEL3_WIDE, F_PANEL3_RB2K, F_PANEL3_KSW, F_PANEL3_KLOOP,
    F_BLEND_SKIN_FWD, F_SKIN_FWD,
    F_SKIN_BWD_VEC, F_SKIN_BWD_SMALL, F_SKIN_BWD_SMALL_K, F_SKIN_BWD_FRAME, F_SKIN_BWD_CHUNKS_MFMA, F_SKIN_BWD_CHUNKS_LIST,
    F_NN_STREAM_W4, F_NN_STREAM_W2, F_NN_STREAM_W1, F_NN_MFMA, F_NN_DIRECT,
    F_VPOSER_SPLIT, F_VPOSER_FP32,
    F_COUNT
};
inline const char* form_name(Form f) {
    static const char* const names[F_COUNT] = {
        nullptr,
        "panel_gemm3_kernel", "panel_gemm3_rb2_kernel", "panel_gemm3_wide_kernel", "panel_gemm3_rb2k_kernel", "panel_gemm3_ksw_kernel",
        "panel_gemm3_kloop_kernel",
        "blend_skin_fwd_kernel", "skin_fwd_kernel",
        "skin_bwd_vec_kernel", "skin_bwd_small_kernel", "skin_bwd_small_kernel(K > 4)", "skin_bwd_kernel(one workgroup per frame)",
        "skin_bwd_kernel(chunks, MFMA dA)", "skin_bwd_kernel(chunks, list dA)",
        "nn_stream4_kernel(4 waves per group)", "nn_stream4_kernel(2 waves per group)", "nn_stream4_kernel<1,1,1>", "nn_mfma_kernel",
        "nn_direct_kernel",
        nullptr, nullptr,
    };
    return names[f];
}


constexpr int PN_SC_U4 = 4 + 4 * 12;
constexpr FDC_FORMS_HD int pn_img_u4(int np, int kpad) { return np * (kpad >> 3) * 16 + PN_SC_U4; }
constexpr FDC_FORMS_HD size_t pn_lds_bytes(int np, int kpad, int rb) { return (size_t)rb * pn_img_u4(np, kpad) * 16; }
constexpr int PN3_MAX_K = 2528;
static_assert(pn_lds_bytes(2, PN3_MAX_K, 1) <= 160 * 1024, "one image per CU");
constexpr bool panel_gemm3_fits(int K) { return ((K + 31) & ~31) <= PN3_MAX_K; }
constexpr size_t pn_b_bytes(int np, int ntile, int nst) { return (size_t)ntile * nst * np * 1024; }

struct PnMap { int nrb, ncb, xc, rpg, cpg, rfast; };
inline PnMap panel_map(int nrb, int ncb, size_t a_bytes, size_t b_bytes) {
    PnMap best{nrb, ncb, 1, (nrb + 7) / 8, ncb, 0};
    double best_cost = 1e300;
    for (int xc = 1; xc <= 8; xc *= 2) {
        const int xr = 8 / xc;
        const int rpg = (nrb + xr - 1) / xr, cpg = (ncb + xc - 1) / xc;
        double cost = (double)xc * a_bytes + ((b_bytes / xc <= (size_t)(3u << 19)) ? 0.0 : (double)xr * b_bytes);
        cost *= (double)(8 * rpg * cpg) / (double)(nrb * ncb);
        if (cost < best_cost) { best_cost = cost; best = PnMap{nrb, ncb, xc, rpg, cpg, 0}; }
    }
    best.rfast = b_bytes / best.xc > (size_t)(3u << 19);
    return best;
}

constexpr int PN3_KLOOP_SLAB = 24;
constexpr int PN3_KLOOP_RB = 2, PN3_KLOOP_T = 2;
inline int panel_gemm3_kloop_parts(int M, int ntile) {
    constexpr int rb = PN3_KLOOP_RB, T = PN3_KLOOP_T, wgs = 256;
    const int ncb = (ntile + 8 * T - 1) / (8 * T), nrp = (M + 16 * rb - 1) / (16 * rb);
    int ks = std::min(64, std::max(1, wgs / (ncb * nrp)));
    while (ks > 1 && (ks * ncb) % 8 != 0) --ks;
    if ((ks * ncb) % 8 != 0) { ks = 1; while ((ks * ncb) % 8 != 0 && ks < 64) ++ks; }
    return std::min(ks, 64);
}

struct PanelPlan {
    Form form = F_NONE;
    int nw = 0, T = 0, cs = 0, ks = 0;
    int grid = 0, block = 0;
// ... 193 lines not shown
```

### 4dcapture-fpv_amd/csrc/fdc_k_skin.h

```cpp
#pragma once

namespace {

__global__ __launch_bounds__(256) void skin_fwd_kernel(SkinModel sm, int nv, const float* __restrict__ X, int ldx, int beta_off, int transl_off,
                                const float* __restrict__ Voff, const float* __restrict__ A,
                                const float* __restrict__ M, const float* __restrict__ scale, int row0, int world,
                                float* __restrict__ Vout, int clip_n = 0, const ClipRow* __restrict__ ctab = nullptr) {
    __shared__ __attribute__((aligned(16))) float sA[NJ * 12];
    const int c = blockIdx.x * 256 + threadIdx.x, cc = min(c, nv - 1);
    const int r = row0 + blockIdx.y;
    glds_wg<1, 4, 16>(A + (size_t)r * NJ * 12, sA, NJ * 3);
    const float* x = X + (size_t)r * ldx;
    const V3 transl = v3(x[transl_off], x[transl_off + 1], x[transl_off + 2]);
    float Mr[12] = {1, 0, 0, 0, 0, 1, 0, 0, 0, 0, 1, 0};
    if (world) {
#pragma unroll
        for (int e = 0; e < 12; ++e) Mr[e] = M[(size_t)r * 12 + e];
    }
    const float sc_v = world ? scale[clip_of_row(r, clip_n, ctab)] : 1.f;
    float* o = Vout + ((size_t)r * nv + c) * 3;
    if (sm.vpack && !FDC_SKIN_HAS_S(sm)) {
        const float4* const vp4 = (const float4*)sm.vpack;
        const int G = (sm.K + 3) >> 2;
        const float4 p0 = vp4[cc], p1 = vp4[nv + cc];
        float4 p2 = make_float4(0.f, 0.f, 0.f, 0.f), p3 = p2, pj = p2;
        if (G >= 2) { p2 = vp4[(size_t)2 * nv + cc]; pj = vp4[(size_t)(G + 1) * nv + cc]; }
        if (G >= 3) p3 = vp4[(size_t)3 * nv + cc];
        const float* vo = Voff + ((size_t)r * nv + cc) * 3;
        const float v0 = vo[0], v1 = vo[1], v2 = vo[2];
        __syncthreads();
        if (c >= nv) return;
        const float px = p0.x + v0, py = p0.y + v1, pz = p0.z + v2;
        const unsigned jb[3] = {__float_as_uint(p0.w), __float_as_uint(pj.x), __float_as_uint(pj.y)};
        const float w12[12] = {p1.x, p1.y, p1.z, p1.w, p2.x, p2.y, p2.z, p2.w, p3.x, p3.y, p3.z, p3.w};
        float T[12];
#pragma unroll
        for (int e = 0; e < 12; ++e) T[e] = 0.f;
#pragma unroll
        for (int k = 0; k < 12; ++k)
            if (k < sm.K) {
                const float* a = sA + 12 * ((jb[k >> 2] >> (8 * (k & 3))) & 255u);
#pragma unroll
                for (int e = 0; e < 12; ++e) T[e] += w12[k] * a[e];
            }
        const V3 vb = v3(T[0] * px + T[1] * py + T[2] * pz + T[3], T[4] * px + T[5] * py + T[6] * pz + T[7],
                         T[8] * px + T[9] * py + T[10] * pz + T[11]) + transl;
        const V3 sv = sc_v * vb;
        o[0] = Mr[0] * sv.x + Mr[1] * sv.y + Mr[2] * sv.z + Mr[3];
        o[1] = Mr[4] * sv.x + Mr[5] * sv.y + Mr[6] * sv.z + Mr[7];
        o[2] = Mr[8] * sv.x + Mr[9] * sv.y + Mr[10] * sv.z + Mr[11];
        return;
    }
    __syncthreads();
    if (c >= nv) return;
    SkinFwd f = skin_forward_vertex(sm, c, x + beta_off, Voff + ((size_t)r * nv + c) * 3, sA, transl, Mr, sc_v);
    o[0] = f.vw.x; o[1] = f.vw.y; o[2] = f.vw.z;
}


__global__ __launch_bounds__(768) void blend_skin_fwd_kernel(const float* __restrict__ PF, int M, PanelB3 B, SkinModel sm, int nv, int ja,
                                                             const float* __restrict__ X, int ldx, int transl_off,
                                                             const float* __restrict__ A, const float* __restrict__ Mw,
                                                             const float* __restrict__ scale, int row0, float* __restrict__ Voff,
                                                             float* __restrict__ Vw, int clip_n = 0,
                                                             const ClipRow* __restrict__ ctab = nullptr) {
    extern __shared__ __attribute__((aligned(16))) uint4 bs_lds[];
    const int tid = threadIdx.x, wave = tid >> 6, lane = tid & 63, j = lane & 15, g = lane >> 4;
    const int cb = blockIdx.x & 7, m0 = (int)(blockIdx.x >> 3) * 32;
    const int ncb = (B.ntile + 11) / 12;
    if (cb >= ncb) return;
    constexpr int K = NPFX, kpad = (NPFX + 31) & ~31, nst = kpad >> 5, pstride = (kpad >> 3) * 16;
    const int img = pnf_img_u4(kpad);
    float* const sA = (float*)(bs_lds + 2 * img);
    float* const sM = sA + 32 * ja * 12;
    float* const sT = sM + 32 * 12;
    float* const sVP = sT + 32 * 4;
    float* const sX = sVP + 2 * 64 * 4;
    const float* const PFr = PF + (size_t)row0 * NPFX;
    PnRing<PnF, 1, 2> rg;
    const int tile = cb * 12 + wave;
    panel_prefetch<PnF, 1, 2>(rg, {B.f + (size_t)min(tile, B.ntile - 1) * B.nst * PNF * 64}, nst, lane);
    const f32x4_t ts = PnF::tile_isc(B, tile, g);
    {
        const int nu = 32 * ja * 3;
        for (int u0 = 0; u0 < nu; u0 += 768) {
            const int u = u0 + tid;
            if (u < nu) {
                const int f = u / (3 * ja), w = u - f * 3 * ja;
                const float* src = A + (size_t)(row0 + min(m0 + f, M - 1)) * NJ * 12 + 4 * w;
                __builtin_amdgcn_global_load_lds((fdc_gptr_t)src, (fdc_lptr_t)((char*)sA + 16 * (u0 + 64 * wave)), 16, 0, 0);
            }
        }
        if (tid < 96) {
            const int f = tid / 3, w = tid - 3 * f;
            const float* src = Mw + (size_t)(row0 + min(m0 + f, M - 1)) * 12 + 4 * w;
            __builtin_amdgcn_global_load_lds((fdc_gptr_t)src, (fdc_lptr_t)((char*)sM + 16 * 64 * wave), 16, 0, 0);
        } else if (tid >= 128 && tid < 128 + 128) {
            const int q = tid - 128, f = q >> 2, w = min(q & 3, 2);
            const float* src = X + (size_t)(row0 + min(m0 + f, M - 1)) * ldx + transl_off + w;
            __builtin_amdgcn_global_load_lds((fdc_gptr_t)src, (fdc_lptr_t)((char*)sT + 4 * 64 * (wave - 2)), 4, 0, 0);
        } else if (tid >= 256 && tid < 256 + 128) {
            const int q = tid - 256;
            const float* src = sm.vpack + 4 * ((size_t)(q >> 6) * nv + min(cb * 64 + (q & 63), nv - 1));
            __builtin_amdgcn_global_load_lds((fdc_gptr_t)src, (fdc_lptr_t)((char*)sVP + 16 * 64 * (wave - 4)), 16, 0, 0);
        }
    }
    const int vv = tid & 63, v = cb * 64 + vv;
    const int clip_lo = clip_of_row(row0 + m0, clip_n, ctab);
    const bool one_clip = clip_of_row(row0 + min(m0 + 31, M - 1), clip_n, ctab) == clip_lo;
    const float sc_v = scale[clip_lo];
    PnF::stage<768, 2, 2>(bs_lds, img, PFr, NPFX, m0, M, 0, K, kpad, tid);
    __syncthreads();
    PnF::Acc acc[2] = {PnF::zero(), PnF::zero()};
    if (tile < B.ntile) panel_mma<PnF, 2, 1, 2, PnOrder::StaticPinLds>(bs_lds, {pstride, img}, rg, nst, acc, lane);
    {
        const int c = wave % 3, vg = wave / 3;
#pragma unroll
        for (int rb = 0; rb < 2; ++rb) {
            const f32x4_t o = PnF::value(acc[rb], PnF::row_isc(bs_lds + (size_t)rb * img, pstride, j), ts);
            *(float4*)(sX + (size_t)((c * 32 + 16 * rb + j) * 64 + vg * 16 + 4 * g)) = make_float4(o[0], o[1], o[2], o[3]);
        }
    }
    __syncthreads();
#pragma unroll
    for (int k = 0; k < 3; ++k) {
        const int p = tid + 768 * k, f = p >> 6;
        if (f < 32 && m0 + f < M && v < nv) {
            const size_t r = (size_t)(row0 + m0 + f);
            const float v0 = sX[(0 * 32 + f) * 64 + vv], v1 = sX[(1 * 32 + f) * 64 + vv], v2 = sX[(2 * 32 + f) * 64 + vv];
            const float4 p0 = ((const float4*)sVP)[vv], p1 = ((const float4*)sVP)[64 + vv];
            float* const vo = Voff + (r * nv + v) * 3;
            vo[0] = v0; vo[1] = v1; vo[2] = v2;
            const float px = p0.x + v0, py = p0.y + v1, pz = p0.z + v2;
            const unsigned jb = __float_as_uint(p0.w);
            const float w4[4] = {p1.x, p1.y, p1.z, p1.w};
            float T[12];
#pragma unroll
            for (int e = 0; e < 12; ++e) T[e] = 0.f;
#pragma unroll
            for (int kk = 0; kk < 4; ++kk)
                if (kk < sm.K) {
                    const float* a = sA + (size_t)(f * ja + (int)((jb >> (8 * kk)) & 255u)) * 12;
#pragma unroll
                    for (int e = 0; e < 12; ++e) T[e] += w4[kk] * a[e];
                }
            const V3 transl = v3(sT[4 * f], sT[4 * f + 1], sT[4 * f + 2]);
            const V3 vb = v3(T[0] * px + T[1] * py + T[2] * pz + T[3], T[4] * px + T[5] * py + T[6] * pz + T[7],
                             T[8] * px + T[9] * py + T[10] * pz + T[11]) + transl;
            const V3 sv = (one_clip ? sc_v : scale[ctab ? ctab[r].k : clip_of_row((int)r, clip_n)]) * vb;
            const float* Mr = sM + 12 * f;
            float* const o = Vw + (r * nv + v) * 3;
            o[0] = Mr[0] * sv.x + Mr[1] * sv.y + Mr[2] * sv.z + Mr[3];
            o[1] = Mr[4] * sv.x + Mr[5] * sv.y + Mr[6] * sv.z + Mr[7];
            o[2] = Mr[8] * sv.x + Mr[9] * sv.y + Mr[10] * sv.z + Mr[11];
        }
    }
}

__device__ __forceinline__ float wave_sum(float v) { return wave_sum64(v); }

struct ContactGradIn { const float* Vw; const float* dist; const int* idx; const float4* scene; const float4* nnpt; float coef; float* loss_rows; };
constexpr int SKB_NACC = NBETA + 3 + 12 + 1;
constexpr int SKP_STRIDE = 688;
static_assert(NJ * 12 + SKB_NACC + 1 <= SKP_STRIDE, "partial record");
#ifndef FDC_SKB_WFQ
#define FDC_SKB_WFQ 4
#endif
constexpr int SKB_WFQ = FDC_SKB_WFQ;
__device__ __forceinline__ SkinFwd skin_forward_vertex_packed(const float4 p0, const float4 p1, int K, const float* __restrict__ voff,
                                                              const float* sA , V3 transl, const float* M, float scale) {
    SkinFwd r;
    const float px = p0.x + voff[0], py = p0.y + voff[1], pz = p0.z + voff[2];
    r.vp = v3(px, py, pz);
    const unsigned jb = __float_as_uint(p0.w);
    const float w4[4] = {p1.x, p1.y, p1.z, p1.w};
#pragma unroll
    for (int e = 0; e < 12; ++e) r.T[e] = 0.f;
#pragma unroll
    for (int k = 0; k < 4; ++k)
        if (k < K) {
            const float4* a = (const float4*)(sA + 12 * ((jb >> (8 * k)) & 255u));
            const float4 a0 = a[0], a1 = a[1], a2 = a[2];
            const float w = w4[k];
            r.T[0] += w * a0.x; r.T[1] += w * a0.y; r.T[2] += w * a0.z; r.T[3] += w * a0.w;
            r.T[4] += w * a1.x; r.T[5] += w * a1.y; r.T[6] += w * a1.z; r.T[7] += w * a1.w;
            r.T[8] += w * a2.x; r.T[9] += w * a2.y; r.T[10] += w * a2.z; r.T[11] += w * a2.w;
        }
    const V3 vl = v3(r.T[0] * px + r.T[1] * py + r.T[2] * pz + r.T[3], r.T[4] * px + r.T[5] * py + r.T[6] * pz + r.T[7],
                     r.T[8] * px + r.T[9] * py + r.T[10] * pz + r.T[11]);
    r.vb = vl + transl;
    const V3 sv = scale * r.vb;
    r.vw = v3(M[0] * sv.x + M[1] * sv.y + M[2] * sv.z + M[3], M[4] * sv.x + M[5] * sv.y + M[6] * sv.z + M[7],
              M[8] * sv.x + M[9] * sv.y + M[10] * sv.z + M[11]);
    return r;
}

#ifndef FDC_SKB_OCC
#define FDC_SKB_OCC 5
#endif
#ifndef FDC_SKB_PACKED
#define FDC_SKB_PACKED 1
#endif
template <bool CONTACT, bool SPLIT = false>
__global__ __launch_bounds__(256, FDC_SKB_OCC) void skin_bwd_kernel(SkinModel sm, int nc, const float* __restrict__ X,
                                                       const float* __restrict__ Voff, const float* __restrict__ A,
                                                       const float* __restrict__ M, const float* __restrict__ scale,
                                                       int row0, const float* dVw, float* dVoff,
                                                       float* __restrict__ dA, float* __restrict__ dbeta_v,
                                                       float* __restrict__ dtransl_v, float* __restrict__ dMv,
                                                       float* __restrict__ dsv, ContactGradIn cg, float* __restrict__ part = nullptr,
                                                       int clip_n = 0, const ClipRow* __restrict__ ctab = nullptr) {
    constexpr int VCH = SKB_VCH;
    extern __shared__ float sdT[];
    __shared__ float sdA[NJ * 12];
    __shared__ float sred[4][SKB_NACC];
    const int tid = threadIdx.x, wave = tid >> 6, lane = tid & 63;
    const int r = row0 + blockIdx.x;
    FDC_FR_STAMP(2, 0);
    const float* x = X + (size_t)r * XDIM;
    int clip_k = clip_of_row(r, clip_n);
    float ccoef = cg.coef;
    if (ctab) { const clip_row_cptr cr = clip_row_at(ctab, r); clip_k = cr->k; ccoef = cr->coef; }
    const float s = scale[clip_k];
    V3 transl = v3(x[X_TRANSL], x[X_TRANSL + 1], x[X_TRANSL + 2]);
    float acc[SKB_NACC];
    float cterm = 0.f;
    const int jlo = lane < NJ ? sm.csc_start[lane] : 0, jhi = lane < NJ ? sm.csc_start[lane + 1] : 0;
    __shared__ __attribute__((aligned(16))) float sAf[NJ * 12];
    __shared__ float sM[12];
    for (int i = tid; i < NJ * 12; i += 256) sAf[i] = A[(size_t)r * NJ * 12 + i];
    if (tid < 12) sM[tid] = M[(size_t)r * 12 + tid];
    const bool packed = FDC_SKB_PACKED && sm.vpack && sm.K <= 4;
    const float4* const vp4 = (const float4*)sm.vpack;
#pragma unroll
    for (int i = 0; i < SKB_NACC; ++i) acc[i] = 0.f;
    for (int i = tid; i < NJ * 12; i += 256) sdA[i] = 0.f;
    __syncthreads();
    FDC_FR_STAMP(2, 1);
    const int c_lo = SPLIT ? (int)blockIdx.y * VCH : 0, c_hi = SPLIT ? min(nc, c_lo + VCH) : nc;
    for (int c0 = c_lo; c0 < c_hi; c0 += VCH) {
        const int c1 = min(c_hi, c0 + VCH);
        for (int c = c0 + tid; c < c1; c += 256) {
            size_t qi = (size_t)r * nc + c;
            float dq = 0.f, vwx = 0.f, vwy = 0.f, vwz = 0.f;
// ... 315 lines not shown
        }
    }
    __syncthreads();
    FDC_FR_STAMP(2, 2);
    {
        const int jlo = lane < NJ ? sCS[lane] : 0, jhi = lane < NJ ? sCS[lane + 1] : 0;
        unsigned long long jact = __ballot(jhi > jlo);
        for (int kact = 0; jact; ++kact) {
            const int j = __ffsll((long long)jact) - 1;
            jact &= jact - 1;
            if ((kact & 3) != wave) continue;
            const int lo = __builtin_amdgcn_readlane(jlo, j), hi = __builtin_amdgcn_readlane(jhi, j);
            float pa[12];
#pragma unroll
            for (int e = 0; e < 12; ++e) pa[e] = 0.f;
            for (int i = lo + lane; i < hi; i += 64) {
                const float w = sCW[i];
                const int v = sCV[i];
                const float gx = w * sGV[3 * v], gy = w * sGV[3 * v + 1], gz = w * sGV[3 * v + 2];
                const float px = sVP[3 * v], py = sVP[3 * v + 1], pz = sVP[3 * v + 2];
                pa[0] += gx * px; pa[1] += gx * py; pa[2] += gx * pz; pa[3] += gx;
                pa[4] += gy * px; pa[5] += gy * py; pa[6] += gy * pz; pa[7] += gy;
                pa[8] += gz * px; pa[9] += gz * py; pa[10] += gz * pz; pa[11] += gz;
            }
#pragma unroll
            for (int e = 0; e < 12; ++e) {
                const float v = wave_sum(pa[e]);
                if (lane == 0) sdA[j * 12 + e] = v;
            }
        }
    }
    FDC_FR_STAMP(2, 3);
#pragma unroll
    for (int i = NBETA; i < SKB_NACC; ++i) {
        const float v = wave_sum(acc[i]);
        if (lane == 0) sred[wave][i] = v;
    }
    const float ct = (cg.loss_rows != nullptr) ? wave_sum(cterm) : 0.f;
    if (cg.loss_rows && lane == 0) sred[wave][0] = ct;
    __syncthreads();
    if (cg.loss_rows && tid == 0) cg.loss_rows[(size_t)r * LROW + 3] = (sred[0][0] + sred[1][0]) + (sred[2][0] + sred[3][0]);
    for (int i = tid; i < sm.ja_hi * 12; i += 256) dA[(size_t)r * NJ * 12 + i] = sdA[i];
    if (tid >= NBETA && tid < SKB_NACC) {
        const float v = sred[0][tid] + sred[1][tid] + sred[2][tid] + sred[3][tid];
        if (tid < NBETA + 3) dtransl_v[(size_t)r * 3 + tid - NBETA] = v;
        else if (tid < NBETA + 15) dMv[(size_t)r * 12 + tid - NBETA - 3] = v;
        else dsv[r] = v;
    }
    FDC_FR_STAMP(2, 4);
}

template <int G>
__global__ __launch_bounds__(256) void skin_bwd_vec_kernel(SkinModel sm, int nc, int nnz, const float* __restrict__ X,
                                                           const float* __restrict__ Voff, const float* __restrict__ A,
                                                           const float* __restrict__ M, const float* __restrict__ scale,
                                                           int row0, float* __restrict__ dVoff, float* __restrict__ dA,
                                                           float* __restrict__ dtransl_v, float* __restrict__ dMv,
                                                           float* __restrict__ dsv, ContactGradIn cg, int clip_n = 0,
                                                           const ClipRow* __restrict__ ctab = nullptr) {
    extern __shared__ __attribute__((aligned(16))) float sk_lds[];
    const int nnz4 = (nnz + 3) & ~3, nnz8 = (nnz + 7) & ~7;
    float* const sGV = sk_lds;
    float* const sVP = sGV + 3 * nc;
    float* const sDV = sVP + 3 * nc;
    float* const sCW = sDV + 3 * nc;
    unsigned short* const sCV = (unsigned short*)(sCW + nnz4);
    __shared__ __attribute__((aligned(16))) float sAf[NJ * 12];
    __shared__ float sdA[NJ * 12];
    __shared__ float sred[4][SKB_NACC];
    __shared__ int sCS[NJ + 1];
    const int tid = threadIdx.x, wave = tid >> 6, lane = tid & 63;
    const int r = row0 + blockIdx.x;
    FDC_FR_STAMP(2, 0);
    const float* x = X + (size_t)r * XDIM;
    int clip_k = clip_of_row(r, clip_n);
    float ccoef = cg.coef;
    if (ctab) { const clip_row_cptr cr = clip_row_at(ctab, r); clip_k = cr->k; ccoef = cr->coef; }
    const float s = scale[clip_k];
    const V3 transl = v3(x[X_TRANSL], x[X_TRANSL + 1], x[X_TRANSL + 2]);
    float Mr[12];
#pragma unroll
    for (int e = 0; e < 12; ++e) Mr[e] = M[(size_t)r * 12 + e];
    const int n4 = (3 * nc) >> 2, nw4 = nnz4 >> 2, nv8 = nnz8 >> 3;
    glds_wg<2, 4, 16>(cg.Vw + (size_t)r * nc * 3, sGV, n4);
    glds_wg<2, 4, 16>(Voff + (size_t)r * nc * 3, sVP, n4);
    glds_wg<2 * G, 4, 16>(sm.csc_w, sCW, nw4);
    glds_wg<G, 4, 16>(sm.csc_v16, sCV, nv8);
    glds_wg<1, 4, 16>(A + (size_t)r * NJ * 12, sAf, NJ * 3);
    glds_wg<1, 4, 4>(sm.csc_start, sCS, NJ + 1);
    float4 lvp0[2], lvp1[2][G], lvpj[2], lpq[2];
    float ldq[2];
    int ljq[2];
#pragma unroll
    for (int k = 0; k < 2; ++k) {
        const int c = min(tid + 256 * k, nc - 1);
        const size_t qi = (size_t)r * nc + c;
        lvp0[k] = ((const float4*)sm.vpack)[c];
#pragma unroll
        for (int g = 0; g < G; ++g) lvp1[k][g] = ((const float4*)sm.vpack)[(size_t)(1 + g) * nc + c];
        lvpj[k] = G > 1 ? ((const float4*)sm.vpack)[(size_t)(1 + G) * nc + c] : make_float4(0.f, 0.f, 0.f, 0.f);
        ldq[k] = cg.dist[qi];
        lpq[k] = cg.nnpt ? cg.nnpt[qi] : make_float4(0.f, 0.f, 0.f, 0.f);
        ljq[k] = cg.nnpt ? __float_as_int(lpq[k].w) : cg.idx[qi];
    }
    for (int i = tid; i < NJ * 12; i += 256) sdA[i] = 0.f;
    __syncthreads();
    FDC_FR_STAMP(2, 1);
    float acc[SKB_NACC];
#pragma unroll
    for (int i = 0; i < SKB_NACC; ++i) acc[i] = 0.f;
    float cterm = 0.f;
#pragma unroll
    for (int u = 0; u < 2; ++u) {
        const int c = tid + 256 * u;
        if (c < nc) {
            SkinFwd f;
            const float p0 = lvp0[u].x + sVP[3 * c], p1 = lvp0[u].y + sVP[3 * c + 1], p2 = lvp0[u].z + sVP[3 * c + 2];
            const float vwx = sGV[3 * c], vwy = sGV[3 * c + 1], vwz = sGV[3 * c + 2];
            f.vp = v3(p0, p1, p2);
#pragma unroll
            for (int e = 0; e < 12; ++e) f.T[e] = 0.f;
            const unsigned jb[3] = {__float_as_uint(lvp0[u].w), __float_as_uint(lvpj[u].x), __float_as_uint(lvpj[u].y)};
#pragma unroll
            for (int k = 0; k < 4 * G; ++k) {
                if (k < sm.K) {
                    const float4 wq = lvp1[u][k >> 2];
                    const float w = (k & 3) == 0 ? wq.x : (k & 3) == 1 ? wq.y : (k & 3) == 2 ? wq.z : wq.w;
                    const float* a = sAf + 12 * ((jb[k >> 2] >> (8 * (k & 3))) & 255u);
#pragma unroll
                    for (int e = 0; e < 12; ++e) f.T[e] += w * a[e];
                }
            }
            const V3 vl = v3(f.T[0] * p0 + f.T[1] * p1 + f.T[2] * p2 + f.T[3], f.T[4] * p0 + f.T[5] * p1 + f.T[6] * p2 + f.T[7],
                             f.T[8] * p0 + f.T[9] * p1 + f.T[10] * p2 + f.T[11]);
            f.vb = vl + transl;
            float dterm;
            cterm += contact_term(ldq[u], &dterm);
            const float gg = ljq[u] >= 0 ? 2.f * ccoef * dterm : 0.f;
            float4 pt = lpq[u];
            if (!cg.nnpt && ljq[u] >= 0) pt = cg.scene[ljq[u]];
            if (ljq[u] < 0) pt = make_float4(0.f, 0.f, 0.f, 0.f);
            const V3 g = v3(gg * (vwx - pt.x), gg * (vwy - pt.y), gg * (vwz - pt.z));
            const SkinBwd b = skin_backward_vertex(f, Mr, s, g);
            sDV[3 * c] = b.dvp.x; sDV[3 * c + 1] = b.dvp.y; sDV[3 * c + 2] = b.dvp.z;
            acc[NBETA] += b.gv.x; acc[NBETA + 1] += b.gv.y; acc[NBETA + 2] += b.gv.z;
#pragma unroll
            for (int e = 0; e < 12; ++e) acc[NBETA + 3 + e] += b.dM[e];
            acc[NBETA + 15] += b.ds;
            sGV[3 * c] = b.gv.x; sGV[3 * c + 1] = b.gv.y; sGV[3 * c + 2] = b.gv.z;
            sVP[3 * c] = p0; sVP[3 * c + 1] = p1; sVP[3 * c + 2] = p2;
        }
    }
    __syncthreads();
    FDC_FR_STAMP(2, 2);
    {
        float4* const gD = (float4*)(dVoff + (size_t)r * nc * 3);
        for (int i = tid; i < n4; i += 256) gD[i] = ((const float4*)sDV)[i];
    }
    {
        const int jlo = lane < NJ ? sCS[lane] : 0, jhi = lane < NJ ? sCS[lane + 1] : 0;
        unsigned long long jact = __ballot(jhi > jlo);
        for (int kact = 0; jact; ++kact) {
            const int j = __ffsll((long long)jact) - 1;
            jact &= jact - 1;
            if ((kact & 3) != wave) continue;
            const int lo = __builtin_amdgcn_readlane(jlo, j), hi = __builtin_amdgcn_readlane(jhi, j);
            float pa[12];
#pragma unroll
            for (int e = 0; e < 12; ++e) pa[e] = 0.f;
            for (int i = lo + lane; i < hi; i += 64) {
                const float w = sCW[i];
                const int v = sCV[i];
                const float gx = w * sGV[3 * v], gy = w * sGV[3 * v + 1], gz = w * sGV[3 * v + 2];
                const float px = sVP[3 * v], py = sVP[3 * v + 1], pz = sVP[3 * v + 2];
                pa[0] += gx * px; pa[1] += gx * py; pa[2] += gx * pz; pa[3] += gx;
                pa[4] += gy * px; pa[5] += gy * py; pa[6] += gy * pz; pa[7] += gy;
                pa[8] += gz * px; pa[9] += gz * py; pa[10] += gz * pz; pa[11] += gz;
            }
#pragma unroll
            for (int e = 0; e < 12; ++e) {
                const float v = wave_sum(pa[e]);
                if (lane == 0) sdA[j * 12 + e] = v;
            }
        }
    }
    FDC_FR_STAMP(2, 3);
#pragma unroll
    for (int i = NBETA; i < SKB_NACC; ++i) {
        const float v = wave_sum(acc[i]);
        if (lane == 0) sred[wave][i] = v;
    }
    const float ct = (cg.loss_rows != nullptr) ? wave_sum(cterm) : 0.f;
    if (cg.loss_rows && lane == 0) sred[wave][0] = ct;
    __syncthreads();
    if (cg.loss_rows && tid == 0) cg.loss_rows[(size_t)r * LROW + 3] = (sred[0][0] + sred[1][0]) + (sred[2][0] + sred[3][0]);
    for (int i = tid; i < sm.ja_hi * 12; i += 256) dA[(size_t)r * NJ * 12 + i] = sdA[i];
    if (tid >= NBETA && tid < SKB_NACC) {
        const float v = sred[0][tid] + sred[1][tid] + sred[2][tid] + sred[3][tid];
        if (tid < NBETA + 3) dtransl_v[(size_t)r * 3 + tid - NBETA] = v;
        else if (tid < NBETA + 15) dMv[(size_t)r * 12 + tid - NBETA - 3] = v;
        else dsv[r] = v;
    }
    FDC_FR_STAMP(2, 4);
}

}
```

### 4dcapture-fpv_amd/csrc/fdc_math.h

```cpp
#pragma once
#include <math.h>

#if defined(__HIPCC__)
#define FDC_HD __host__ __device__ __forceinline__
#else
#define FDC_HD inline
#endif

namespace fdc {

struct FormLog { const char* name[48]; int n; };
inline FormLog& form_log() { static FormLog f{}; return f; }
inline void note_form(const char* name) {
    FormLog& f = form_log();
    for (int i = 0; i < f.n; ++i) if (f.name[i] == name || !__builtin_strcmp(f.name[i], name)) return;
    if (f.n < 48) f.name[f.n++] = name;
}

#if defined(__HIPCC__)
template <int CTRL>
__device__ __forceinline__ float dpp_move(float v) {
    return __int_as_float(__builtin_amdgcn_update_dpp(0, __float_as_int(v), CTRL, 0xF, 0xF, false));
}
__device__ __forceinline__ float wave_sum64(float v) {
    v += dpp_move<0xB1>(v);
    v += dpp_move<0x4E>(v);
    v += dpp_move<0x141>(v);
    v += dpp_move<0x140>(v);
    v += __int_as_float(__builtin_amdgcn_update_dpp(0, __float_as_int(v), 0x142, 0x2, 0xF, false));
    v += __int_as_float(__builtin_amdgcn_update_dpp(0, __float_as_int(v), 0x142, 0x4, 0xF, false));
    v += __int_as_float(__builtin_amdgcn_update_dpp(0, __float_as_int(v), 0x142, 0x8, 0xF, false));
    return __int_as_float(__builtin_amdgcn_readlane(__float_as_int(v), 63));
}
__device__ __forceinline__ float wave_min64(float v) {
    v = fminf(v, dpp_move<0xB1>(v)); v = fminf(v, dpp_move<0x4E>(v)); v = fminf(v, dpp_move<0x141>(v)); v = fminf(v, dpp_move<0x140>(v));
    const float r0 = __int_as_float(__builtin_amdgcn_readlane(__float_as_int(v), 0));
    const float r1 = __int_as_float(__builtin_amdgcn_readlane(__float_as_int(v), 16));
    const float r2 = __int_as_float(__builtin_amdgcn_readlane(__float_as_int(v), 32));
    const float r3 = __int_as_float(__builtin_amdgcn_readlane(__float_as_int(v), 48));
    return fminf(fminf(r0, r1), fminf(r2, r3));
}
__device__ __forceinline__ float wave_max64(float v) { return -wave_min64(-v); }
#endif

struct V3 { float x, y, z; };
struct M3 { float m[9]; };

FDC_HD V3 v3(float x, float y, float z) { V3 r; r.x = x; r.y = y; r.z = z; return r; }
FDC_HD V3 operator+(V3 a, V3 b) { return v3(a.x + b.x, a.y + b.y, a.z + b.z); }
FDC_HD V3 operator-(V3 a, V3 b) { return v3(a.x - b.x, a.y - b.y, a.z - b.z); }
FDC_HD V3 operator*(float s, V3 a) { return v3(s * a.x, s * a.y, s * a.z); }
FDC_HD float dot(V3 a, V3 b) { return a.x * b.x + a.y * b.y + a.z * b.z; }
FDC_HD V3 cross(V3 a, V3 b) {
    return v3(a.y * b.z - a.z * b.y, a.z * b.x - a.x * b.z, a.x * b.y - a.y * b.x);
}
FDC_HD M3 m3_zero() { M3 r; for (int i = 0; i < 9; ++i) r.m[i] = 0.f; return r; }
FDC_HD M3 m3_identity() { M3 r = m3_zero(); r.m[0] = r.m[4] = r.m[8] = 1.f; return r; }
FDC_HD M3 m3_mul(const M3& a, const M3& b) {
    M3 r;
    for (int i = 0; i < 3; ++i)
        for (int j = 0; j < 3; ++j)
            r.m[3 * i + j] = a.m[3 * i] * b.m[j] + a.m[3 * i + 1] * b.m[3 + j] + a.m[3 * i + 2] * b.m[6 + j];
    return r;
}
FDC_HD M3 m3_mul_bt(const M3& a, const M3& b) {
    M3 r;
    for (int i = 0; i < 3; ++i)
        for (int j = 0; j < 3; ++j)
            r.m[3 * i + j] = a.m[3 * i] * b.m[3 * j] + a.m[3 * i + 1] * b.m[3 * j + 1] + a.m[3 * i + 2] * b.m[3 * j + 2];
    return r;
}
FDC_HD M3 m3_mul_at(const M3& a, const M3& b) {
    M3 r;
    for (int i = 0; i < 3; ++i)
        for (int j = 0; j < 3; ++j)
            r.m[3 * i + j] = a.m[i] * b.m[j] + a.m[3 + i] * b.m[3 + j] + a.m[6 + i] * b.m[6 + j];
    return r;
}
FDC_HD V3 m3_vec(const M3& a, V3 v) {
    return v3(a.m[0] * v.x + a.m[1] * v.y + a.m[2] * v.z,
              a.m[3] * v.x + a.m[4] * v.y + a.m[5] * v.z,
              a.m[6] * v.x + a.m[7] * v.y + a.m[8] * v.z);
}
FDC_HD V3 m3t_vec(const M3& a, V3 v) {
    return v3(a.m[0] * v.x + a.m[3] * v.y + a.m[6] * v.z,
              a.m[1] * v.x + a.m[4] * v.y + a.m[7] * v.z,
              a.m[2] * v.x + a.m[5] * v.y + a.m[8] * v.z);
}
FDC_HD void m3_add_outer(M3& r, V3 a, V3 b) {
    r.m[0] += a.x * b.x; r.m[1] += a.x * b.y; r.m[2] += a.x * b.z;
    r.m[3] += a.y * b.x; r.m[4] += a.y * b.y; r.m[5] += a.y * b.z;
    r.m[6] += a.z * b.x; r.m[7] += a.z * b.y; r.m[8] += a.z * b.z;
}
FDC_HD void m3_add(M3& r, const M3& a) { for (int i = 0; i < 9; ++i) r.m[i] += a.m[i]; }

struct GsCache { V3 b1, b2, a2; float n1, n2, d; };

FDC_HD M3 gs_forward(const float* s, int stride, GsCache* c) {
    V3 a1 = v3(s[0], s[2 * stride], s[4 * stride]);
    V3 a2 = v3(s[stride], s[3 * stride], s[5 * stride]);
    float n1 = fmaxf(sqrtf(dot(a1, a1)), 1e-12f);
    V3 b1 = (1.f / n1) * a1;
    float d = dot(b1, a2);
    V3 u = a2 - d * b1;
    float n2 = fmaxf(sqrtf(dot(u, u)), 1e-12f);
    V3 b2 = (1.f / n2) * u;
    V3 b3 = cross(b1, b2);
    M3 R;
    R.m[0] = b1.x; R.m[1] = b2.x; R.m[2] = b3.x;
    R.m[3] = b1.y; R.m[4] = b2.y; R.m[5] = b3.y;
    R.m[6] = b1.z; R.m[7] = b2.z; R.m[8] = b3.z;
    if (c) { c->b1 = b1; c->b2 = b2; c->a2 = a2; c->n1 = n1; c->n2 = n2; c->d = d; }
    return R;
}

FDC_HD void gs_backward(const GsCache& c, const M3& dR, float* ds, int stride) {
    V3 db1 = v3(dR.m[0], dR.m[3], dR.m[6]);
    V3 db2 = v3(dR.m[1], dR.m[4], dR.m[7]);
    V3 db3 = v3(dR.m[2], dR.m[5], dR.m[8]);
    db1 = db1 + cross(c.b2, db3);
    db2 = db2 + cross(db3, c.b1);
    V3 du = (1.f / c.n2) * (db2 - dot(c.b2, db2) * c.b2);
    V3 da2 = du;
    float dd = -dot(du, c.b1);
    db1 = db1 - c.d * du;
    db1 = db1 + dd * c.a2;
// ... 131 lines not shown
```

### 4dcapture-fpv_amd/csrc/fdc_skin.h

```cpp
#pragma once
#include "fdc_math.h"

namespace fdc {

struct SkinModel {
    const float* vt;
    const float* S;
    const int* wj;
    const float* ww;
    int K;
    const int* csc_start;
    const int* csc_v;
    const float* csc_w;
    const float* vpack = nullptr;
    const unsigned short* csc_v16 = nullptr;
    const int* csc_chunk = nullptr;
    int nch = 0;
    int ja_hi = 55;
    const int* wf_tab = nullptr;
    const unsigned* wf_step = nullptr;
    const float* wf_frag = nullptr;
};

#ifdef __HIP_DEVICE_COMPILE__
#define FDC_SKIN_HAS_S(sm) false
#else
#define FDC_SKIN_HAS_S(sm) ((sm).S != nullptr)
#endif

FDC_HD int skin_vpack_planes(int K) { const int G = (K + 3) / 4; return G <= 1 ? 2 : G + 2; }

struct SkinFwd { V3 vp, vb, vw; float T[12]; };

FDC_HD SkinFwd skin_forward_vertex(const SkinModel& sm, int v, const float* beta, const float* voff,
                                   const float* A, V3 transl, const float* M, float scale) {
    SkinFwd r;
    float p[3];
    for (int c = 0; c < 3; ++c) {
        float acc = sm.vt[3 * v + c];
        if (FDC_SKIN_HAS_S(sm)) {
            const float* s = sm.S + (3 * v + c) * 10;
            for (int l = 0; l < 10; ++l) acc += s[l] * beta[l];
        }
        p[c] = acc + voff[c];
    }
    r.vp = v3(p[0], p[1], p[2]);
    for (int e = 0; e < 12; ++e) r.T[e] = 0.f;
    for (int k = 0; k < sm.K; ++k) {
        float w = sm.ww[v * sm.K + k];
        const float* a = A + 12 * sm.wj[v * sm.K + k];
        for (int e = 0; e < 12; ++e) r.T[e] += w * a[e];
    }
    V3 vl = v3(r.T[0] * p[0] + r.T[1] * p[1] + r.T[2] * p[2] + r.T[3],
               r.T[4] * p[0] + r.T[5] * p[1] + r.T[6] * p[2] + r.T[7],
               r.T[8] * p[0] + r.T[9] * p[1] + r.T[10] * p[2] + r.T[11]);
    r.vb = vl + transl;
    V3 sv = scale * r.vb;
    r.vw = v3(M[0] * sv.x + M[1] * sv.y + M[2] * sv.z + M[3],
              M[4] * sv.x + M[5] * sv.y + M[6] * sv.z + M[7],
              M[8] * sv.x + M[9] * sv.y + M[10] * sv.z + M[11]);
    return r;
}

struct SkinBwd { float dT[12]; V3 dvp, gv; float dM[12]; float ds; };

FDC_HD SkinBwd skin_backward_vertex(const SkinFwd& f, const float* M, float scale, V3 g) {
    SkinBwd b;
    V3 sv = scale * f.vb;
    b.dM[0] = g.x * sv.x; b.dM[1] = g.x * sv.y; b.dM[2] = g.x * sv.z;  b.dM[3] = g.x;
    b.dM[4] = g.y * sv.x; b.dM[5] = g.y * sv.y; b.dM[6] = g.y * sv.z;  b.dM[7] = g.y;
    b.dM[8] = g.z * sv.x; b.dM[9] = g.z * sv.y; b.dM[10] = g.z * sv.z; b.dM[11] = g.z;
    V3 gs = v3(M[0] * g.x + M[4] * g.y + M[8] * g.z,
               M[1] * g.x + M[5] * g.y + M[9] * g.z,
               M[2] * g.x + M[6] * g.y + M[10] * g.z);
    b.ds = dot(gs, f.vb);
    b.gv = scale * gs;
    b.dT[0] = b.gv.x * f.vp.x; b.dT[1] = b.gv.x * f.vp.y; b.dT[2] = b.gv.x * f.vp.z;  b.dT[3] = b.gv.x;
    b.dT[4] = b.gv.y * f.vp.x; b.dT[5] = b.gv.y * f.vp.y; b.dT[6] = b.gv.y * f.vp.z;  b.dT[7] = b.gv.y;
    b.dT[8] = b.gv.z * f.vp.x; b.dT[9] = b.gv.z * f.vp.y; b.dT[10] = b.gv.z * f.vp.z; b.dT[11] = b.gv.z;
    b.dvp = v3(f.T[0] * b.gv.x + f.T[4] * b.gv.y + f.T[8] * b.gv.z,
               f.T[1] * b.gv.x + f.T[5] * b.gv.y + f.T[9] * b.gv.z,
               f.T[2] * b.gv.x + f.T[6] * b.gv.y + f.T[10] * b.gv.z);
    return b;
}

FDC_HD float contact_term(float d, float* dterm_dd) {
    float r = sqrtf(d + 1e-4f);
    float q = 1.f / (r + 1.f);
    *dterm_dd = q * q * (0.5f / r);
    return r * q;
}

}
```

### 4dcapture-fpv_amd/csrc/fdc_state.h

```cpp
#pragma once

namespace {

struct SetupTrace {
    bool on;
    const char* who;
    std::chrono::steady_clock::time_point t0, last;
    explicit SetupTrace(const char* w) : who(w) {
        const char* e = getenv("FDCAP_SETUP_TRACE");
        on = e && e[0] == '1';
        if (on) t0 = last = std::chrono::steady_clock::now();
    }
    void mark(const char* what) {
        if (!on) return;
        (void)hipDeviceSynchronize();
        const auto now = std::chrono::steady_clock::now();
        fprintf(stderr, "[fdcap setup] %s: %-28s %8.3f ms (at %8.3f)\n", who, what, std::chrono::duration<double, std::milli>(now - last).count(),
                std::chrono::duration<double, std::milli>(now - t0).count());
        last = now;
    }
};

template <class T>
struct DevBuf {
// ... 34 lines not shown
                       CONTACT ? cg.loss_rows : (float*)nullptr);
    return (int)hipGetLastError();
}

struct SkinSet {
    int nv = 0, K = 0, nnz = 0;
    int ldp = 0;
    DevBuf<float> vt, ww, posedirs, csc_w;
    DevBuf<int> wj, csc_start, csc_v, csc_chunk;
    int nch = 0, ja_hi = NJ;
    DevBuf<int> wf_tab; DevBuf<uint2> wf_step; DevBuf<float4> wf_frag;
    DevBuf<float4> vpack;
    DevBuf<unsigned short> csc_v16;
    DevBuf<float> pn_fwd_f, pn_bwd_f;
    PanelB pn_fwd, pn_bwd;
    DevBuf<unsigned> pn_fwd3_f, pn_bwd3_f;
    DevBuf<float> pn_fwd3_s, pn_bwd3_s;
    DevBuf<unsigned> pn_fwdS_f; DevBuf<float> pn_fwdS_s; PanelB3 pn_fwdS;
    PanelB3 pn_fwd3, pn_bwd3;
    SkinModel model() const {
        SkinModel m; m.vt = vt.p; m.S = nullptr; m.wj = wj.p; m.ww = ww.p; m.K = K;
        m.csc_start = csc_start.p; m.csc_v = csc_v.p; m.csc_w = csc_w.p;
        m.vpack = (const float*)vpack.p; m.csc_v16 = csc_v16.p;
        m.csc_chunk = csc_chunk.p; m.nch = nch; m.ja_hi = ja_hi;
        m.wf_tab = wf_tab.p; m.wf_step = (const unsigned*)wf_step.p; m.wf_frag = (const float*)wf_frag.p;
        return m;
    }
    void release() { vt.release(); ww.release(); posedirs.release(); wj.release(); csc_w.release(); csc_start.release(); csc_v.release();
                     vpack.release(); csc_v16.release(); csc_chunk.release(); wf_tab.release(); wf_step.release(); wf_frag.release();
                     pn_fwd_f.release(); pn_bwd_f.release(); pn_fwd = PanelB(); pn_bwd = PanelB();
                     pn_fwd3_f.release(); pn_bwd3_f.release(); pn_fwd3_s.release(); pn_bwd3_s.release(); pn_fwdS_f.release(); pn_fwdS_s.release(); pn_fwdS = PanelB3(); pn_fwd3 = PanelB3(); pn_bwd3 = PanelB3(); }
};

struct OptState {
    fdcap_opt_config cfg;
    int R = 0;
    int nclip = 1, clip_len = 0;
    bool ragged = false;
    std::vector<int32_t> clip_lens, clip_start;
    DevBuf<ClipRow> clip_rows;
    DevBuf<int> clip_span;
    const ClipRow* ctab(bool phase2) const { return ragged ? clip_rows.p + (phase2 ? (size_t)R : 0) : nullptr; }
    const int* cspan() const { return ragged ? clip_span.p : nullptr; }
    int kclip_n() const { return nclip > 1 ? clip_len : 0; }
    int rows_per_clip() const { return ragged ? 1 : cfg.n_local / nclip; }
    bool contact_on = false;
    int nsplit = 8;
    int nsplit_bf = 8;
    struct Ext { float* p = nullptr; } X, CAM, scale, dscale;
    struct ExtD { double* p = nullptr; } losses;
    DevBuf<float> X0, mask, mX, vX, mCAM, vCAM, mS, vS;
    struct { bool on = false; int ii = 0, P = 0; } pend;
    DevBuf<float> H1, H2, O, dO;
    DevBuf<float> Opart, dZpart;
    bool dz_pending = false;
    DevBuf<float> Rm, PF, Jrest, G, A, M, Jw;
    PoseJoints pj_fwd, pj_bwd;
    DevBuf<float> Voff, Vw, dist, pd, dVoff;
    DevBuf<int> idx, pi;
    DevBuf<float> kp2d;
    DevBuf<float> floss;
    fdcap_lbfgs* lbfgs = nullptr;
    DevBuf<float4> seedpt;
    FormSwitches sw;
    DevBuf<float> loss_rows;
    bool log_pending = false;
    unsigned log_mask = 0;
    int log_assign = 0;
    double* log_dst = nullptr;
    DevBuf<unsigned short> nnc_ids;
    DevBuf<int> nnc_hdr;
    DevBuf<float4> nnc_anchor;
    DevBuf<int> nnq_buf;
    NNOrder nn_order;
    struct LaunchTimes {
        bool on = false;
        int used = 0, phase = 0;
        std::vector<hipEvent_t> ev;
        std::vector<signed char> what;
    } lt;
    bool nn_timing = false;
    std::vector<hipEvent_t> nn_ev;
    int nn_ev_used = 0;
    NNCache nn_cache(int) { return NNCache{sw.nn_cache_slack > 0.f ? nnc_ids.p : nullptr, sw.nn_cache_slack > 0.f ? nnc_hdr.p : nullptr, nnc_anchor.p, sw.nn_cache_slack}; }
    DevBuf<float> dA, dtransl_v, dMv, dsv, dPF, dJw, dX, dCAM, dscale_row;
    DevBuf<float> VoffF, VwF, dVF;
    int cam_steps = 0;
    DevBuf<float> dctD, dctCoef, dctM, dctV;
    DevBuf<AdamScalars> adam_tab;
    std::vector<AdamScalars> adam_tab_h;
    int dctT = 0, dctC = 0, dctW = 0;
    bool dct_grad = false;
    bool seeded = false;
    bool ahead = false, ahead_blend = false;
    bool nnpt_valid = false;
};

inline void lt_mark(OptState* o, int what, hipStream_t st) {
    OptState::LaunchTimes& t = o->lt;
    if (!t.on || t.used >= (int)t.ev.size()) return;
    if (hipEventRecord(t.ev[t.used], st) != hipSuccess) return;
    t.what[t.used++] = (signed char)(what < 0 ? -1 : what + 16 * t.phase);
}

}

struct fdcap_lbfgs {
    int n = 0;
    LbfgsCfg cf{};
    DevBuf<LbfgsScalars> S;
    DevBuf<float> W, RO;
    DevBuf<int> active;
    int* active_h = nullptr;
    int round = 0;
};

struct fdcap_ctx {
    int V = 0;
    std::vector<float> h_vt, h_S10, h_lbs;
    DevBuf<float> d_posedirs, d_S10;
    DevBuf<float> Jt, Jd, hand_comp, hand_mean;
    DevBuf<int> parents, order, level_start, child_start, child_list, depth;
    DevBuf<float> pose_tab;
    int nlevels = 0;
    std::vector<int> h_parents, h_depth;
    DevBuf<float> W1, b1, W2, b2, W3, b3;
    DevBuf<float> vp_pn[6];
    VPoserPanels vp;
    DevBuf<unsigned> vp_pn3[6];
    DevBuf<float> vp_pn3s[6];
    VPoserPanels3 vp3;
    SkinSet full, contact;
    bool full_ready = false;
    DevBuf<float4> scene;
    DevBuf<float4> scene_sorted;
    DevBuf<float4> scene_bounds;
    DevBuf<float4> scene_sbounds;
    DevBuf<float4> scene_qbounds;
    DevBuf<int> scene_inv;
    DevBuf<uint4> scene_frags;
    DevBuf<float4> scene_centers;
    int64_t ns = 0;
    NNTarget nn_target(bool cull) const {
        NNTarget t; t.pts = scene_sorted.p; t.n = (int)ns; t.bounds = cull ? scene_bounds.p : nullptr; t.inv_perm = scene_inv.p;
        t.sbounds = cull ? scene_sbounds.p : nullptr; t.qbounds = cull ? scene_qbounds.p : nullptr;
        t.frags = cull ? scene_frags.p : nullptr; t.centers = scene_centers.p;
        return t;
    }
    int nc = 0;
    DevBuf<int> contact_vid;
    DevBuf<int> contact_perm;
    DevBuf<AdamScalars> ws_adam;
    std::vector<AdamScalars> ws_adam_h;
    DevBuf<float> ws_f[12];
    DevBuf<float> ws_b[12];
    DevBuf<float> ws_part;
    DevBuf<int> ws_i[2];
    DevBuf<float4> ws_p;
    DevBuf<float> ws_skin;
    DevBuf<float> ws_kpart;
    struct SceneOp {
        DevBuf<float> dist;
        DevBuf<int> idx, hdr;
        DevBuf<float4> seedpt, anchor;
        DevBuf<unsigned short> ids;
        int nq = 0;
        void release() { dist.release(); idx.release(); hdr.release(); seedpt.release(); anchor.release(); ids.release(); nq = 0; }
    } sop;
    OptState* opt = nullptr;
    Comm comm;
    DevBuf<float> xch_send, xch_all;
    std::string comm_err;

    PoseModel pose_model() const {
        PoseModel pm;
        pm.tab = pose_tab.p;
        pm.Jt = Jt.p; pm.Jd = Jd.p; pm.parents = parents.p; pm.order = order.p; pm.level_start = level_start.p;
        pm.child_start = child_start.p; pm.child_list = child_list.p; pm.hand_comp = hand_comp.p;
// ... 68 lines not shown
    return (int)e;
}

int build_skin_set(fdcap_ctx* c, const std::vector<int64_t>& ids, SkinSet* out) {
    SetupTrace tr("build_skin_set");
    const int V = c->V;
    const int nv = (int)ids.size();
    int K = 1;
    for (int v : ids) {
        int k = 0;
        for (int j = 0; j < NJ; ++j) k += c->h_lbs[(size_t)v * NJ + j] != 0.f;
        K = std::max(K, k);
    }
    const int ldp = (3 * nv + 3) & ~3;
    std::vector<float> vt((size_t)nv * 3), ww((size_t)nv * K, 0.f);
    std::vector<int> wj((size_t)nv * K, 0);
    for (int i = 0; i < nv; ++i) {
        int64_t v = ids[i];
        for (int k = 0; k < 3; ++k) vt[3 * i + k] = c->h_vt[3 * v + k];
        int k = 0;
        for (int j = 0; j < NJ; ++j) {
            float w = c->h_lbs[(size_t)v * NJ + j];
            if (w != 0.f) { wj[(size_t)i * K + k] = j; ww[(size_t)i * K + k] = w; ++k; }
        }
    }
    const size_t pd_floats = (size_t)NPFX * ldp;
    HIP_TRY(out->posedirs.ensure(pd_floats));
    {
        std::vector<int> id32((size_t)std::max(nv, 1), 0);
        for (int i = 0; i < nv; ++i) id32[i] = (int)ids[i];
        DevBuf<int> d_ids;
        { hipError_t eu = d_ids.upload(id32.data(), id32.size()); if (eu != hipSuccess) { d_ids.release(); return (int)eu; } }
        if (ldp > 0) hipLaunchKernelGGL(blend_rows_gather_kernel, dim3((ldp + 255) / 256, NPFX), dim3(256), 0, 0, c->d_posedirs.p, c->d_S10.p, V, d_ids.p, nv, ldp, out->posedirs.p);
        hipError_t e_ = hipGetLastError();
        if (e_ == hipSuccess) e_ = hipDeviceSynchronize();
        d_ids.release();
        HIP_TRY(e_);
    }
    const float* pd = out->posedirs.p;
    tr.mark("gather vt / weights / posedirs");
    std::vector<int> csc_start(NJ + 1, 0), csc_v;
    std::vector<float> csc_w;
    for (int j = 0; j < NJ; ++j) {
        csc_start[j] = (int)csc_v.size();
        for (int i = 0; i < nv; ++i) {
            float w = c->h_lbs[(size_t)ids[i] * NJ + j];
            if (w != 0.f) { csc_v.push_back(i); csc_w.push_back(w); }
        }
    }
    csc_start[NJ] = (int)csc_v.size();
    out->nnz = (int)csc_v.size();
    if (csc_v.empty()) { csc_v.push_back(0); csc_w.push_back(0.f); }
    while (csc_w.size() & 3) csc_w.push_back(0.f);
    out->nv = nv; out->K = K; out->ldp = ldp;
    out->vpack.release(); out->csc_v16.release();
    if (K <= 12 && nv > 0 && nv <= 65535) {
        const int G = (K + 3) / 4, NP = skin_vpack_planes(K);
        std::vector<float4> vp((size_t)nv * NP);
        for (int i = 0; i < nv; ++i) {
            unsigned jb[3] = {0, 0, 0};
            float w12[12] = {0.f};
            for (int k = 0; k < K; ++k) { jb[k >> 2] |= (unsigned)wj[(size_t)i * K + k] << (8 * (k & 3)); w12[k] = ww[(size_t)i * K + k]; }
            float jf[3]; memcpy(jf, jb, 12);
            vp[(size_t)i] = make_float4(vt[3 * i], vt[3 * i + 1], vt[3 * i + 2], jf[0]);
            for (int g = 0; g < G; ++g) vp[(size_t)(1 + g) * nv + i] = make_float4(w12[4 * g], w12[4 * g + 1], w12[4 * g + 2], w12[4 * g + 3]);
            if (G > 1) vp[(size_t)(1 + G) * nv + i] = make_float4(jf[1], jf[2], 0.f, 0.f);
        }
        std::vector<unsigned short> v16((csc_v.size() + 7) & ~(size_t)7, 0);
        for (size_t i = 0; i < csc_v.size(); ++i) v16[i] = (unsigned short)csc_v[i];
        HIP_TRY(out->vpack.upload(vp.data(), vp.size()));
        HIP_TRY(out->csc_v16.upload(v16.data(), v16.size()));
    }
    {
        const int nch = std::max(1, (nv + SKB_VCH - 1) / SKB_VCH);
        std::vector<int> cc((size_t)NJ * (nch + 1), 0);
        for (int j = 0; j < NJ; ++j) {
            int i = csc_start[j];
            for (int ch = 0; ch <= nch; ++ch) {
                while (i < csc_start[j + 1] && csc_v[i] < ch * SKB_VCH) ++i;
                cc[(size_t)j * (nch + 1) + ch] = ch == nch ? csc_start[j + 1] : i;
            }
        }
        out->nch = nch;
        out->ja_hi = 1;
        for (int j = 0; j < NJ; ++j) if (csc_start[j + 1] > csc_start[j]) out->ja_hi = j + 1;
        HIP_TRY(out->csc_chunk.upload(cc.data(), cc.size()));
    }
    tr.mark("lists, vpack, chunk table");
    out->wf_tab.release(); out->wf_step.release(); out->wf_frag.release();
    {
        if (nv > 512) {
            const int nchm = (nv + SKB_VCH - 1) / SKB_VCH;
            std::vector<int> tab((size_t)nchm * 16 + 1, 0);
            std::vector<uint2> steps;
            std::vector<float4> frag;
            for (int ch = 0; ch < nchm; ++ch)
                for (int q = 0; q < 4; ++q)
                    for (int jt = 0; jt < 4; ++jt) {
                        tab[((size_t)ch * 4 + q) * 4 + jt] = (int)steps.size();
                        std::vector<int> st;
                        std::vector<float> fr;
                        for (int s = 64 * q; s < 64 * q + 64; ++s) {
                            const int v0 = ch * SKB_VCH + 4 * s;
                            if (v0 >= nv) break;
                            float f[64];
                            bool any = false;
                            for (int l = 0; l < 64; ++l) f[l] = 0.f;
                            for (int kk = 0; kk < 4 && v0 + kk < nv; ++kk)
                                for (int k = 0; k < K; ++k) {
                                    const int j = wj[(size_t)(v0 + kk) * K + k];
                                    const float w = ww[(size_t)(v0 + kk) * K + k];
                                    if (w != 0.f && (j >> 4) == jt) { f[16 * kk + (j & 15)] += w; any = true; }
                                }
                            if (any) { st.push_back(s); fr.insert(fr.end(), f, f + 64); }
                        }
                        while (st.size() & 3) { st.push_back(st.empty() ? 0 : st.back()); fr.insert(fr.end(), 64, 0.f); }
                        for (size_t g = 0; g < st.size(); g += 4) {
                            steps.push_back(make_uint2((unsigned)st[g] | ((unsigned)st[g + 1] << 16), (unsigned)st[g + 2] | ((unsigned)st[g + 3] << 16)));
                            for (int l = 0; l < 64; ++l)
                                frag.push_back(make_float4(fr[(g + 0) * 64 + l], fr[(g + 1) * 64 + l], fr[(g + 2) * 64 + l], fr[(g + 3) * 64 + l]));
                        }
                    }
            tab.back() = (int)steps.size();
            if (steps.empty()) { steps.push_back(make_uint2(0u, 0u)); frag.resize(64, make_float4(0.f, 0.f, 0.f, 0.f)); }
            HIP_TRY(out->wf_tab.upload(tab.data(), tab.size()));
            HIP_TRY(out->wf_step.upload(steps.data(), steps.size()));
            HIP_TRY(out->wf_frag.upload(frag.data(), frag.size()));
        }
    }
    tr.mark("weight fragments");
    HIP_TRY(out->csc_start.upload(csc_start.data(), csc_start.size()));
    HIP_TRY(out->csc_v.upload(csc_v.data(), csc_v.size()));
    HIP_TRY(out->csc_w.upload(csc_w.data(), csc_w.size()));
    HIP_TRY(out->vt.upload(vt.data(), vt.size()));
    HIP_TRY(out->ww.upload(ww.data(), ww.size()));
    HIP_TRY(out->wj.upload(wj.data(), wj.size()));
    tr.mark("uploads");
    out->pn_fwd = PanelB(); out->pn_bwd = PanelB();
    if (nv > 0) {
        int nt = 0, ns = 0;
        int e = panel_pack_dev(pd, pd_floats, ldp, 1, NPFX, 3 * nv, out->pn_fwd_f, &nt, &ns);
        if (e) return e;
        out->pn_fwd.f = (const float4*)out->pn_fwd_f.p; out->pn_fwd.ntile = nt; out->pn_fwd.nss = ns;
    }
    if (nv > 0 && 3 * nv <= PANEL_MAX_K) {
        int nt = 0, ns = 0;
        int e = panel_pack_dev(pd, pd_floats, 1, ldp, 3 * nv, NPFX, out->pn_bwd_f, &nt, &ns);
        if (e) return e;
        out->pn_bwd.f = (const float4*)out->pn_bwd_f.p; out->pn_bwd.ntile = nt; out->pn_bwd.nss = ns;
    }
    tr.mark("fp32 panels");
    out->pn_fwd3 = PanelB3(); out->pn_bwd3 = PanelB3();
    if (nv > 0) {
        int e = pnf_pack_dev(pd, pd_floats, ldp, 1, NPFX, 3 * nv, out->pn_fwd3_f, out->pn_fwd3_s, &out->pn_fwd3.ntile, &out->pn_fwd3.nst);
        if (e) return e;
        out->pn_fwd3.f = (const uint4*)out->pn_fwd3_f.p; out->pn_fwd3.isc = out->pn_fwd3_s.p;
    }
    tr.mark("split forward panel");
    out->pn_fwdS = PanelB3();
    if (nv > 0 && nv <= 512 && K <= 4) {
        const int nb = (nv + 63) / 64, ncs = nb * 192;
        DevBuf<float> ps;
        { hipError_t ep = ps.ensure((size_t)NPFX * ncs); if (ep != hipSuccess) return (int)ep; }
        hipLaunchKernelGGL(blend_rows_permute_kernel, dim3((ncs + 255) / 256, NPFX), dim3(256), 0, 0, pd, ldp, nv, ncs, ps.p);
        int e = (int)hipGetLastError();
        if (!e) e = pnf_pack_dev(ps.p, (size_t)NPFX * ncs, ncs, 1, NPFX, ncs, out->pn_fwdS_f, out->pn_fwdS_s, &out->pn_fwdS.ntile, &out->pn_fwdS.nst);
        if (!e) e = (int)hipDeviceSynchronize();
        ps.release();
// ... 192 lines not shown
```

### include/fdcap.h

```cpp
#ifndef FDCAP_H
#define FDCAP_H

#include <stdint.h>

#ifdef __cplusplus
extern "C" {
#endif

#define FDCAP_OK 0
#define FDCAP_E_ARG (-1)
#define FDCAP_E_STATE (-2)
#define FDCAP_E_NODEVICE (-3)
#define FDCAP_E_COMM (-4)
#define FDCAP_UNIQUE_ID_BYTES 128

#define FDCAP_NUM_JOINTS 55
#define FDCAP_XDIM 78
#define FDCAP_PDIM 75
#define FDCAP_MAX_SCENE_POINTS 67000000
#define FDCAP_NUM_LOSSES 8

typedef struct fdcap_ctx fdcap_ctx;

typedef struct fdcap_model_desc {
// ... 97 lines not shown
int fdcap_opt_run(fdcap_ctx* ctx, int32_t ii0, int32_t ii1, int32_t num_iter, int32_t first_phase2_iter, int32_t log_every,
                  double* hist_d, int32_t hist_rows, int32_t flags, int32_t* n_logged, void* stream);
int32_t fdcap_opt_state_len(fdcap_ctx* ctx);
int fdcap_opt_export_state(fdcap_ctx* ctx, float* state_d, void* stream);
int fdcap_opt_import_state(fdcap_ctx* ctx, const float* state_d, void* stream);
int fdcap_opt_check_finite(fdcap_ctx* ctx, int32_t* count_d, void* stream);
int fdcap_opt_set_loss_output(fdcap_ctx* ctx, double* losses_d);
int fdcap_opt_detect_contact(fdcap_ctx* ctx, int32_t n_left, float* weight_left_d, void* stream);
int fdcap_opt_backward_local2(fdcap_ctx* ctx, const float* contact_weight_d, int32_t n_left, void* stream);
int fdcap_opt_step_x(fdcap_ctx* ctx, int32_t step, void* stream);

int fdcap_opt_set_dct(fdcap_ctx* ctx, const float* dct_mtx, int32_t T, int32_t C, const float* c_dct_d, void* stream);
int fdcap_opt_dct_fit(fdcap_ctx* ctx, int32_t iters, int32_t step0, float weight, float* obj_hist_d,
                      int32_t log_stride, void* stream);
int fdcap_opt_backward_dct(fdcap_ctx* ctx, float w_dct, float w_rec, float w_contact, int32_t log_terms, void* stream);
int fdcap_opt_set_dct_coef(fdcap_ctx* ctx, const float* c_dct_d, void* stream);
int fdcap_opt_get_dct(fdcap_ctx* ctx, float* c_dct_d, void* stream);
int fdcap_opt_get_dct_state(fdcap_ctx* ctx, float* m_d, float* v_d, void* stream);
int fdcap_opt_set_dct_state(fdcap_ctx* ctx, const float* m_d, const float* v_d, void* stream);
int32_t fdcap_opt_dct_windows(fdcap_ctx* ctx, int32_t* w0, int32_t* w1);

int fdcap_frame_smoother(fdcap_ctx* ctx, const float* data78_d, int32_t N, int32_t iters, float lr, float w_rec,
                         float w_vposer, float w_prev, float* state_d, int32_t step0, int32_t has_prev,
                         float* out78_d, void* stream);

typedef struct fdcap_fit2d_stage {
    float fx, fy, cx, cy;
    float rho;
    float w_data, w_pose, w_shape, w_hand;
} fdcap_fit2d_stage;
int fdcap_opt_set_keypoints(fdcap_ctx* ctx, const float* kp_d, void* stream);
int fdcap_opt_backward_fit2d(fdcap_ctx* ctx, const fdcap_fit2d_stage* stage, int32_t log_terms, void* stream);
int fdcap_opt_reset_adam(fdcap_ctx* ctx, void* stream);

typedef struct fdcap_lbfgs_config {
    int32_t dim, history, max_iter, max_eval, max_steps, max_ls;
    float lr, tolerance_grad, tolerance_change, ftol, gtol;
} fdcap_lbfgs_config;
typedef struct fdcap_lbfgs fdcap_lbfgs;
int fdcap_lbfgs_create(int32_t n_problems, const fdcap_lbfgs_config* cfg, fdcap_lbfgs** out);
void fdcap_lbfgs_destroy(fdcap_lbfgs* opt);
int fdcap_lbfgs_reset(fdcap_lbfgs* opt, void* stream);
int fdcap_lbfgs_advance(fdcap_lbfgs* opt, float* x_d, int32_t x_stride, const float* f_d, const float* g_d, int32_t g_stride,
                        int32_t* n_active_d, void* stream);
int fdcap_lbfgs_finalize(fdcap_lbfgs* opt, float* x_d, int32_t x_stride, int32_t* n_unfinished_d, void* stream);
int fdcap_lbfgs_get_stats(fdcap_lbfgs* opt, int32_t* iterations_d, int32_t* evaluations_d, float* loss_d, void* stream);

int fdcap_opt_fit2d_lbfgs(fdcap_ctx* ctx, const fdcap_fit2d_stage* stage, const fdcap_lbfgs_config* cfg, int32_t max_rounds,
                          int32_t* rounds_out, void* stream);
int fdcap_opt_fit2d_lbfgs_stats(fdcap_ctx* ctx, int32_t* iterations_d, int32_t* evaluations_d, float* loss_d, void* stream);

int fdcap_opt_step_rows_and_pack(fdcap_ctx* ctx, int32_t ii, int32_t first_phase2_iter, float* send_d, void* stream);
int fdcap_opt_unpack_and_step_scale(fdcap_ctx* ctx, int32_t ii, int32_t first_phase2_iter, const float* gathered_d,
                                    int32_t rank, int32_t world, void* stream);
int32_t fdcap_exchange_len(void);

int fdcap_comm_unique_id(uint8_t* id128);
int fdcap_comm_create(fdcap_ctx* ctx, const uint8_t* id128, int32_t rank, int32_t world);
int fdcap_comm_destroy(fdcap_ctx* ctx);
const char* fdcap_comm_last_error(fdcap_ctx* ctx);
int fdcap_opt_halo_exchange(fdcap_ctx* ctx, void* stream);
int fdcap_opt_exchange(fdcap_ctx* ctx, int32_t ii, int32_t first_phase2_iter, void* stream);
int fdcap_opt_time_exchange(fdcap_ctx* ctx, int32_t iters, float* us_exchange, float* us_allgather, void* stream);
int fdcap_comm_allreduce_f64(fdcap_ctx* ctx, double* buf_d, int32_t n, void* stream);
int fdcap_opt_forward_ahead(fdcap_ctx* ctx, int32_t ii, int32_t first_phase2_iter, int32_t log_terms, void* stream);

int fdcap_opt_get_results(fdcap_ctx* ctx, float* body_rec75_d, float* scale_d, float* cam_ext_d,
                          void* stream);
void fdcap_opt_destroy(fdcap_ctx* ctx);

int fdcap_opt_forward_world(fdcap_ctx* ctx, float* verts_d, float* joints_d, void* stream);
int fdcap_opt_get_contact(fdcap_ctx* ctx, float* dist_d, int32_t* idx_d, void* stream);
int fdcap_opt_get_grads(fdcap_ctx* ctx, float* dx_d, float* dcam_d, void* stream);

int fdcap_time_blend_gemm(fdcap_ctx* ctx, int32_t rows, int32_t iters, float* ms, void* stream);

int fdcap_panel_gemm(const float* A_d, int32_t lda, int32_t M, int32_t K, const float* B_h, int64_t sk, int64_t sn, int32_t N,
                     float* C_d, int32_t ldc, void* stream);

int fdcap_opt_nn_timing(fdcap_ctx* ctx, int32_t max_launches);
int fdcap_opt_nn_timing_read(fdcap_ctx* ctx, float* mean_ms, int32_t* launches);

int fdcap_debug_nn_query_order(fdcap_ctx* ctx, int32_t mode, const int32_t* perm_h, int32_t n);

int fdcap_debug_nn_query_sort(fdcap_ctx* ctx, const int32_t* pos_h, int32_t nq, int32_t groups, int32_t hdr_len, int32_t* hdr_io,
                              int32_t* perm_out, void* stream);

#define FDCAP_LT_VPOSER_FWD 0
#define FDCAP_LT_POSE_FWD 1
#define FDCAP_LT_CONTACT_FWD 2
#define FDCAP_LT_CHAMFER_NN 3
#define FDCAP_LT_SKIN_BWD 4
#define FDCAP_LT_BLEND_BWD 5
#define FDCAP_LT_POSE_BWD 6
#define FDCAP_LT_VPOSER_BWD 7
#define FDCAP_LT_NUM 8
int fdcap_opt_launch_timing(fdcap_ctx* ctx, int32_t max_events);
int fdcap_opt_launch_timing_read(fdcap_ctx* ctx, float* mean_us , int32_t* counts );

int fdcap_opt_time_chamfer(fdcap_ctx* ctx, int32_t iters, int32_t brute_force, float* ms, void* stream);

#ifdef __cplusplus
}
#endif
#endif
```

Baseline: 18520 frames/s.

## Skip unchanged NN record writes and recompute contact world verts in skin backward

The nearest-neighbour streaming kernel, in its one-wave-per-block variant, now compares each query's final neighbour with the seed record. It skips rewriting idx and seedpt when they are unchanged, which cuts global stores. The vectorised contact skin-backward kernel can recompute world vertices and squared distances from the skinning transform and the cached neighbour point. This replaces loading Vw and dist, and it limits the A load to ja_hi joints. Both paths are on by default behind environment switches. They trade memory traffic for extra ALU work and a ballot, and they add debug counters and API hooks.

```diff
diff --git a/4dcapture-fpv_amd/capi.py b/4dcapture-fpv_amd/capi.py
--- a/4dcapture-fpv_amd/capi.py
+++ b/4dcapture-fpv_amd/capi.py
@@ -135,6 +135,9 @@
     "fdcap_opt_nn_timing": (c_int32, [c_void_p, c_int32]),
     "fdcap_opt_nn_timing_read": (c_int32, [c_void_p, POINTER(c_float), POINTER(c_int32)]),
     "fdcap_debug_nn_query_order": (c_int32, [c_void_p, c_int32, c_void_p, c_int32]),
+    "fdcap_debug_nn_records": (c_int32, [c_void_p, c_void_p, c_void_p]),
+    "fdcap_debug_contact_diet": (c_int32, [c_void_p, c_void_p]),
+    "fdcap_debug_contact_perm": (c_int32, [c_void_p, c_void_p, c_int32]),
     "fdcap_debug_nn_query_sort": (c_int32, [c_void_p, c_void_p, c_int32, c_int32, c_int32, c_void_p, c_void_p, c_void_p]),
     "fdcap_opt_launch_timing": (c_int32, [c_void_p, c_int32]),
     "fdcap_opt_launch_timing_read": (c_int32, [c_void_p, c_void_p, c_void_p]),
diff --git a/4dcapture-fpv_amd/csrc/fdc_api_opt.h b/4dcapture-fpv_amd/csrc/fdc_api_opt.h
--- a/4dcapture-fpv_amd/csrc/fdc_api_opt.h
+++ b/4dcapture-fpv_amd/csrc/fdc_api_opt.h
@@ -56,6 +56,8 @@
     o->dz_pending = false;
     o->log_pending = false;
     o->seeded = false;
+    o->nnpt_valid = false;
+    o->n_recompute = 0;
     o->dctT = o->dctC = o->dctW = 0;
     o->dct_grad = false;
     const int R = o->R = cfg->n_local + 4;
@@ -63,6 +65,8 @@
     const size_t nq = (size_t)R * std::max(c->nc, 1);
     o->sw = forms_read_env();
     { const char* e = getenv("FDCAP_POSE_TRIM"); o->sw.pose_trim = !(e && e[0] == '0'); }
+    { const char* e = getenv("FDCAP_NN_KEEP_RECORDS"); o->sw.nn_keep_records = !(e && e[0] == '0'); }
+    { const char* e = getenv("FDCAP_CONTACT_RECOMPUTE"); o->sw.contact_recompute = !(e && e[0] == '0'); }
     const int nq_all = (int)((size_t)cfg->n_local * c->nc);
     o->nsplit = o->contact_on ? nn_pick_nsplit(nq_all, (int)c->ns, o->sw.nn_seed && o->sw.nn_cull) : 1;
     o->nsplit_bf = o->contact_on ? nn_pick_nsplit(nq_all, (int)c->ns, false) : 1;
@@ -278,6 +282,8 @@
         const SkinBwdPlan pl = plan_contact_skin_bwd(nl, nc, nnz, smc.K, smc.vpack != nullptr, smc.csc_v16 != nullptr, aligned16, smc.wf_tab != nullptr,
                                                      o->sw.skin_vec);
         if (pl.ja_rows) dA_rows = c->contact.ja_hi;
+        cg.recompute = pl.form == F_SKIN_BWD_VEC && cg.nnpt != nullptr && o->sw.contact_recompute;
+        o->n_recompute += cg.recompute;
         const dim3 grid(pl.grid), block(pl.block);
 #define FDC_SKC(KERNEL) hipLaunchKernelGGL(KERNEL, grid, block, pl.lds, st, smc, nc, nnz, o->X.p, o->Voff.p, o->A.p, o->M.p, o->scale.p, 2, o->dVoff.p, \
                                            o->dA.p, o->dtransl_v.p, o->dMv.p, o->dsv.p, cg, kn, ctab)
diff --git a/4dcapture-fpv_amd/csrc/fdc_api_run.h b/4dcapture-fpv_amd/csrc/fdc_api_run.h
--- a/4dcapture-fpv_amd/csrc/fdc_api_run.h
+++ b/4dcapture-fpv_amd/csrc/fdc_api_run.h
@@ -306,6 +306,30 @@
     if (idx) hipLaunchKernelGGL(unpermute_kernel<int>, dim3((n + 255) / 256), dim3(256), 0, st, o->idx.p + 2 * nc,
                                 c->contact_perm.p, nl, nc, 1, idx);
     return (int)hipGetLastError();
+}
+
+int fdcap_debug_nn_records(fdcap_ctx* c, float* rec4, void* stream) {
+    if (!c || !c->opt || !rec4) return FDCAP_E_STATE;
+    OptState* o = c->opt;
+    if (!o->contact_on || !o->nnpt_valid) return FDCAP_E_STATE;
+    const int nl = o->cfg.n_local, nc = c->nc;
+    const size_t n = (size_t)nl * nc * 4;
+    hipLaunchKernelGGL(unpermute_kernel<float>, dim3((n + 255) / 256), dim3(256), 0, (hipStream_t)stream, (const float*)(o->seedpt.p + 2 * nc),
+                       c->contact_perm.p, nl, nc, 4, rec4);
+    return (int)hipGetLastError();
+}
+
+int fdcap_debug_contact_diet(fdcap_ctx* c, int32_t* out4) {
+    if (!c || !c->opt || !out4) return FDCAP_E_STATE;
+    const OptState* o = c->opt;
+    out4[0] = o->nn_order.n_kept; out4[1] = o->n_recompute; out4[2] = o->nn_order.n_permuted; out4[3] = o->nn_order.n_rebuilds;
+    return FDCAP_OK;
+}
+
+int fdcap_debug_contact_perm(fdcap_ctx* c, int32_t* perm_h, int32_t n) {
+    if (!c || !perm_h || n != c->nc || n <= 0) return FDCAP_E_ARG;
+    HIP_TRY(hipMemcpy(perm_h, c->contact_perm.p, (size_t)n * sizeof(int32_t), hipMemcpyDeviceToHost));
+    return FDCAP_OK;
 }
 
 int fdcap_opt_get_grads(fdcap_ctx* c, float* dx, float* dcam, void* stream) {
diff --git a/4dcapture-fpv_amd/csrc/fdc_chamfer.h b/4dcapture-fpv_amd/csrc/fdc_chamfer.h
--- a/4dcapture-fpv_amd/csrc/fdc_chamfer.h
+++ b/4dcapture-fpv_amd/csrc/fdc_chamfer.h
@@ -22,13 +22,6 @@
     const float4* centers;
 };
 
-__device__ __forceinline__ float nn_exact_d2(float qx, float qy, float qz, float px, float py, float pz) {
-    float dx = qx - px, dy = qy - py, dz = qz - pz;
-    return __fmaf_rn(dz, dz, __fmaf_rn(dy, dy, __fmul_rn(dx, dx)));
-}
-__device__ __forceinline__ bool nn_better(float d, int i, float bd, int bi) {
-    return d < bd || (d == bd && i < bi);
-}
 
 __device__ __forceinline__ void nn_block_map(int b, int nsplit, int* qb, int* split) {
     const int xcd = b & 7, slot = b >> 3;
@@ -396,6 +389,7 @@
     float slack;
     int order_mode = 0;
     const int* perm = nullptr;
+    bool keep = false;
 };
 
 template <int NQ, int WPG, int WPB = 4>
@@ -479,7 +473,7 @@
         qx[n] = ok ? lqx[n] : 0.f;
         qy[n] = ok ? lqy[n] : 0.f;
         qz[n] = ok ? lqz[n] : 0.f;
-        own_d[n] = INFINITY;
+        own_d[n] = NN_NO_NEIGHBOUR_D2;
         own_i[n] = -1;
         own_p[n] = make_float4(0.f, 0.f, 0.f, __int_as_float(-1));
         const int sj = ok ? lsj[n] : -1;
@@ -507,6 +501,15 @@
     }
     const bool cull = __all(all_seeded && finite);
     TL_STAMP(0);
+    constexpr bool KEEP = WPB == 1;
+    if constexpr (KEEP) {
+#pragma unroll
+        for (int n = 0; n < NQ; ++n)
+            if (half == 0) {
+                s_i[wave][n * 32 + col] = (cache.keep && own_i[n] >= 0) ? own_i[n] : -2;
+                s_d[wave][n * 32 + col] = own_p[n].w;
+            }
+    }
     auto min_rows01 = [](float v) {
         v = fminf(v, dpp_move<0xB1>(v)); v = fminf(v, dpp_move<0x4E>(v)); v = fminf(v, dpp_move<0x141>(v)); v = fminf(v, dpp_move<0x140>(v));
         return fminf(__int_as_float(__builtin_amdgcn_readlane(__float_as_int(v), 0)), __int_as_float(__builtin_amdgcn_readlane(__float_as_int(v), 16)));
@@ -913,6 +916,7 @@
     }
     TL_STAMP(3);
     if (cache.order_mode != 0 && lane == 0 && !idle) cache.hdr[4 * ((nq + 31) / 32) + (int)blockIdx.x] = nsurv;
+    unsigned keepm[NQ];
 #pragma unroll
     for (int n = 0; n < NQ; ++n) {
         const float od = __shfl_xor(own_d[n], 32, 64);
@@ -921,6 +925,11 @@
         op.x = __shfl_xor(own_p[n].x, 32, 64); op.y = __shfl_xor(own_p[n].y, 32, 64);
         op.z = __shfl_xor(own_p[n].z, 32, 64); op.w = __shfl_xor(own_p[n].w, 32, 64);
         if (oi >= 0 && (own_i[n] < 0 || nn_better(od, oi, own_d[n], own_i[n]))) { own_d[n] = od; own_i[n] = oi; own_p[n] = op; }
+        keepm[n] = 0u;
+        if constexpr (KEEP) {
+            const bool same = half == 0 && s_i[wave][n * 32 + col] == own_i[n] && __float_as_int(s_d[wave][n * 32 + col]) == __float_as_int(own_p[n].w);
+            keepm[n] = (unsigned)__ballot(same);
+        }
         if (half == 0) { s_d[wave][n * 32 + col] = own_d[n]; s_i[wave][n * 32 + col] = own_i[n]; s_p[wave][n * 32 + col] = own_p[n]; }
     }
     __syncthreads();
@@ -957,8 +966,10 @@
             }
             const int qd = perm ? s_q[g][e] : qo;
             dist[qd] = bd;
-            idx[qd] = bi;
-            seedpt[qd] = s_p[bw][e];
+            if (!KEEP || !((keepm[e >> 5] >> (e & 31)) & 1u)) {
+                idx[qd] = bi;
+                seedpt[qd] = s_p[bw][e];
+            }
         }
     }
 }
@@ -1106,6 +1117,7 @@
     int* qbuf = nullptr;
     int perm_n = 0;
     int perm_mode = 0;
+    int n_kept = 0, n_permuted = 0, n_rebuilds = 0;
 };
 static inline size_t nn_query_order_ints(int nq);
 static inline hipError_t nn_query_order(const float4* seedpt, int nq, int* qbuf, int* hdr, int groups, hipStream_t st);
@@ -1131,6 +1143,8 @@
             nc.order_mode = !ordered ? 0 : (ord->sorted_groups == groups ? 2 + ord->cur : 1);
             const bool qorder = ordered && ord->qbuf != nullptr && ord->perm_mode != 1;
             nc.perm = qorder && ord->perm_n == nq ? ord->qbuf : nullptr;
+            nc.keep = nc.keep && wpg == 1 && seedpt != nullptr && seed != nullptr && seed == idx && !seed_missing;
+            if (ord) { ord->n_kept += nc.keep ? 1 : 0; ord->n_permuted += nc.perm ? 1 : 0; }
             if (wpg == 4) hipLaunchKernelGGL((nn_stream4_kernel<1, 4>), grid, block, 0, st, q, nq, T, seed, seedpt, dist, idx, nc);
             else if (wpg == 2) hipLaunchKernelGGL((nn_stream4_kernel<1, 2>), grid, block, 0, st, q, nq, T, seed, seedpt, dist, idx, nc);
             else hipLaunchKernelGGL((nn_stream4_kernel<1, 1, 1>), grid, block, 0, st, q, nq, T, seed, seedpt, dist, idx, nc);
@@ -1141,6 +1155,7 @@
                 ord->perm_n = nq;
                 ord->sorted_groups = 0;
                 ord->age = 0;
+                ++ord->n_rebuilds;
             } else if (resort) {
                 const bool had = nc.order_mode >= 2;
                 const int nxt = had ? 1 - ord->cur : 0;
diff --git a/4dcapture-fpv_amd/csrc/fdc_forms.h b/4dcapture-fpv_amd/csrc/fdc_forms.h
--- a/4dcapture-fpv_amd/csrc/fdc_forms.h
+++ b/4dcapture-fpv_amd/csrc/fdc_forms.h
@@ -26,6 +26,8 @@
     bool skin_vec = true;
     bool fuse_skin = true;
     bool pose_trim = true;
+    bool nn_keep_records = true;
+    bool contact_recompute = true;
 };
 inline FormSwitches forms_read_env() {
     FormSwitches s;
diff --git a/4dcapture-fpv_amd/csrc/fdc_k_skin.h b/4dcapture-fpv_amd/csrc/fdc_k_skin.h
--- a/4dcapture-fpv_amd/csrc/fdc_k_skin.h
+++ b/4dcapture-fpv_amd/csrc/fdc_k_skin.h
@@ -45,10 +45,8 @@
             }
         const V3 vb = v3(T[0] * px + T[1] * py + T[2] * pz + T[3], T[4] * px + T[5] * py + T[6] * pz + T[7],
                          T[8] * px + T[9] * py + T[10] * pz + T[11]) + transl;
-        const V3 sv = sc_v * vb;
-        o[0] = Mr[0] * sv.x + Mr[1] * sv.y + Mr[2] * sv.z + Mr[3];
-        o[1] = Mr[4] * sv.x + Mr[5] * sv.y + Mr[6] * sv.z + Mr[7];
-        o[2] = Mr[8] * sv.x + Mr[9] * sv.y + Mr[10] * sv.z + Mr[11];
+        const V3 vw = skin_world_vertex(vb, sc_v, Mr);
+        o[0] = vw.x; o[1] = vw.y; o[2] = vw.z;
         return;
     }
     __syncthreads();
@@ -147,19 +145,17 @@
             const V3 transl = v3(sT[4 * f], sT[4 * f + 1], sT[4 * f + 2]);
             const V3 vb = v3(T[0] * px + T[1] * py + T[2] * pz + T[3], T[4] * px + T[5] * py + T[6] * pz + T[7],
                              T[8] * px + T[9] * py + T[10] * pz + T[11]) + transl;
-            const V3 sv = (one_clip ? sc_v : scale[ctab ? ctab[r].k : clip_of_row((int)r, clip_n)]) * vb;
-            const float* Mr = sM + 12 * f;
+            const V3 vw = skin_world_vertex(vb, one_clip ? sc_v : scale[ctab ? ctab[r].k : clip_of_row((int)r, clip_n)], sM + 12 * f);
             float* const o = Vw + (r * nv + v) * 3;
-            o[0] = Mr[0] * sv.x + Mr[1] * sv.y + Mr[2] * sv.z + Mr[3];
-            o[1] = Mr[4] * sv.x + Mr[5] * sv.y + Mr[6] * sv.z + Mr[7];
-            o[2] = Mr[8] * sv.x + Mr[9] * sv.y + Mr[10] * sv.z + Mr[11];
+            o[0] = vw.x; o[1] = vw.y; o[2] = vw.z;
         }
     }
 }
 
 __device__ __forceinline__ float wave_sum(float v) { return wave_sum64(v); }
 
-struct ContactGradIn { const float* Vw; const float* dist; const int* idx; const float4* scene; const float4* nnpt; float coef; float* loss_rows; };
+struct ContactGradIn { const float* Vw; const float* dist; const int* idx; const float4* scene; const float4* nnpt; float coef; float* loss_rows;
+                       int recompute = 0; };
 constexpr int SKB_NACC = NBETA + 3 + 12 + 1;
 constexpr int SKP_STRIDE = 688;
 static_assert(NJ * 12 + SKB_NACC + 1 <= SKP_STRIDE, "partial record");
@@ -641,11 +637,12 @@
 #pragma unroll
     for (int e = 0; e < 12; ++e) Mr[e] = M[(size_t)r * 12 + e];
     const int n4 = (3 * nc) >> 2, nw4 = nnz4 >> 2, nv8 = nnz8 >> 3;
-    glds_wg<2, 4, 16>(cg.Vw + (size_t)r * nc * 3, sGV, n4);
+    const bool recompute = cg.recompute != 0;
+    if (!recompute) glds_wg<2, 4, 16>(cg.Vw + (size_t)r * nc * 3, sGV, n4);
     glds_wg<2, 4, 16>(Voff + (size_t)r * nc * 3, sVP, n4);
     glds_wg<2 * G, 4, 16>(sm.csc_w, sCW, nw4);
     glds_wg<G, 4, 16>(sm.csc_v16, sCV, nv8);
-    glds_wg<1, 4, 16>(A + (size_t)r * NJ * 12, sAf, NJ * 3);
+    glds_wg<1, 4, 16>(A + (size_t)r * NJ * 12, sAf, (recompute ? sm.ja_hi : NJ) * 3);
     glds_wg<1, 4, 4>(sm.csc_start, sCS, NJ + 1);
     float4 lvp0[2], lvp1[2][G], lvpj[2], lpq[2];
     float ldq[2];
@@ -658,7 +655,7 @@
 #pragma unroll
         for (int g = 0; g < G; ++g) lvp1[k][g] = ((const float4*)sm.vpack)[(size_t)(1 + g) * nc + c];
         lvpj[k] = G > 1 ? ((const float4*)sm.vpack)[(size_t)(1 + G) * nc + c] : make_float4(0.f, 0.f, 0.f, 0.f);
-        ldq[k] = cg.dist[qi];
+        ldq[k] = recompute ? 0.f : cg.dist[qi];
         lpq[k] = cg.nnpt ? cg.nnpt[qi] : make_float4(0.f, 0.f, 0.f, 0.f);
         ljq[k] = cg.nnpt ? __float_as_int(lpq[k].w) : cg.idx[qi];
     }
@@ -675,7 +672,8 @@
         if (c < nc) {
             SkinFwd f;
             const float p0 = lvp0[u].x + sVP[3 * c], p1 = lvp0[u].y + sVP[3 * c + 1], p2 = lvp0[u].z + sVP[3 * c + 2];
-            const float vwx = sGV[3 * c], vwy = sGV[3 * c + 1], vwz = sGV[3 * c + 2];
+            float vwx = 0.f, vwy = 0.f, vwz = 0.f;
+            if (!recompute) { vwx = sGV[3 * c]; vwy = sGV[3 * c + 1]; vwz = sGV[3 * c + 2]; }
             f.vp = v3(p0, p1, p2);
 #pragma unroll
             for (int e = 0; e < 12; ++e) f.T[e] = 0.f;
@@ -693,11 +691,17 @@
             const V3 vl = v3(f.T[0] * p0 + f.T[1] * p1 + f.T[2] * p2 + f.T[3], f.T[4] * p0 + f.T[5] * p1 + f.T[6] * p2 + f.T[7],
                              f.T[8] * p0 + f.T[9] * p1 + f.T[10] * p2 + f.T[11]);
             f.vb = vl + transl;
-            float dterm;
-            cterm += contact_term(ldq[u], &dterm);
-            const float gg = ljq[u] >= 0 ? 2.f * ccoef * dterm : 0.f;
             float4 pt = lpq[u];
             if (!cg.nnpt && ljq[u] >= 0) pt = cg.scene[ljq[u]];
+            float dq = ldq[u];
+            if (recompute) {
+                const V3 vw = skin_world_vertex(f.vb, s, Mr);
+                vwx = vw.x; vwy = vw.y; vwz = vw.z;
+                dq = ljq[u] >= 0 ? nn_exact_d2(vwx, vwy, vwz, pt.x, pt.y, pt.z) : NN_NO_NEIGHBOUR_D2;
+            }
+            float dterm;
+            cterm += contact_term(dq, &dterm);
+            const float gg = ljq[u] >= 0 ? 2.f * ccoef * dterm : 0.f;
             if (ljq[u] < 0) pt = make_float4(0.f, 0.f, 0.f, 0.f);
             const V3 g = v3(gg * (vwx - pt.x), gg * (vwy - pt.y), gg * (vwz - pt.z));
             const SkinBwd b = skin_backward_vertex(f, Mr, s, g);
diff --git a/4dcapture-fpv_amd/csrc/fdc_math.h b/4dcapture-fpv_amd/csrc/fdc_math.h
--- a/4dcapture-fpv_amd/csrc/fdc_math.h
+++ b/4dcapture-fpv_amd/csrc/fdc_math.h
@@ -42,6 +42,19 @@
 }
 __device__ __forceinline__ float wave_max64(float v) { return -wave_min64(-v); }
 #endif
+
+FDC_HD float nn_exact_d2(float qx, float qy, float qz, float px, float py, float pz) {
+    float dx = qx - px, dy = qy - py, dz = qz - pz;
+#if defined(__HIP_DEVICE_COMPILE__)
+    return __fmaf_rn(dz, dz, __fmaf_rn(dy, dy, __fmul_rn(dx, dx)));
+#else
+    return fmaf(dz, dz, fmaf(dy, dy, dx * dx));
+#endif
+}
+FDC_HD bool nn_better(float d, int i, float bd, int bi) {
+    return d < bd || (d == bd && i < bi);
+}
+constexpr float NN_NO_NEIGHBOUR_D2 = INFINITY;
 
 struct V3 { float x, y, z; };
 struct M3 { float m[9]; };
diff --git a/4dcapture-fpv_amd/csrc/fdc_skin.h b/4dcapture-fpv_amd/csrc/fdc_skin.h
--- a/4dcapture-fpv_amd/csrc/fdc_skin.h
+++ b/4dcapture-fpv_amd/csrc/fdc_skin.h
@@ -28,9 +28,22 @@
 #define FDC_SKIN_HAS_S(sm) ((sm).S != nullptr)
 #endif
 
+FDC_HD int skin_ja_hi(const int* csc_start, int nj) {
+    int hi = 1;
+    for (int j = 0; j < nj; ++j) if (csc_start[j + 1] > csc_start[j]) hi = j + 1;
+    return hi;
+}
+
 FDC_HD int skin_vpack_planes(int K) { const int G = (K + 3) / 4; return G <= 1 ? 2 : G + 2; }
 
 struct SkinFwd { V3 vp, vb, vw; float T[12]; };
+
+FDC_HD V3 skin_world_vertex(V3 vb, float scale, const float* M) {
+    const V3 sv = scale * vb;
+    return v3(M[0] * sv.x + M[1] * sv.y + M[2] * sv.z + M[3],
+              M[4] * sv.x + M[5] * sv.y + M[6] * sv.z + M[7],
+              M[8] * sv.x + M[9] * sv.y + M[10] * sv.z + M[11]);
+}
 
 FDC_HD SkinFwd skin_forward_vertex(const SkinModel& sm, int v, const float* beta, const float* voff,
                                    const float* A, V3 transl, const float* M, float scale) {
@@ -55,10 +68,7 @@
                r.T[4] * p[0] + r.T[5] * p[1] + r.T[6] * p[2] + r.T[7],
                r.T[8] * p[0] + r.T[9] * p[1] + r.T[10] * p[2] + r.T[11]);
     r.vb = vl + transl;
-    V3 sv = scale * r.vb;
-    r.vw = v3(M[0] * sv.x + M[1] * sv.y + M[2] * sv.z + M[3],
-              M[4] * sv.x + M[5] * sv.y + M[6] * sv.z + M[7],
-              M[8] * sv.x + M[9] * sv.y + M[10] * sv.z + M[11]);
+    r.vw = skin_world_vertex(r.vb, scale, M);
     return r;
 }
 
diff --git a/4dcapture-fpv_amd/csrc/fdc_state.h b/4dcapture-fpv_amd/csrc/fdc_state.h
--- a/4dcapture-fpv_amd/csrc/fdc_state.h
+++ b/4dcapture-fpv_amd/csrc/fdc_state.h
@@ -140,7 +140,11 @@
     bool nn_timing = false;
     std::vector<hipEvent_t> nn_ev;
     int nn_ev_used = 0;
-    NNCache nn_cache(int) { return NNCache{sw.nn_cache_slack > 0.f ? nnc_ids.p : nullptr, sw.nn_cache_slack > 0.f ? nnc_hdr.p : nullptr, nnc_anchor.p, sw.nn_cache_slack}; }
+    NNCache nn_cache(int) {
+        NNCache nc{sw.nn_cache_slack > 0.f ? nnc_ids.p : nullptr, sw.nn_cache_slack > 0.f ? nnc_hdr.p : nullptr, nnc_anchor.p, sw.nn_cache_slack};
+        nc.keep = sw.nn_keep_records;
+        return nc;
+    }
     DevBuf<float> dA, dtransl_v, dMv, dsv, dPF, dJw, dX, dCAM, dscale_row;
     DevBuf<float> VoffF, VwF, dVF;
     int cam_steps = 0;
@@ -152,6 +156,7 @@
     bool seeded = false;
     bool ahead = false, ahead_blend = false;
     bool nnpt_valid = false;
+    int n_recompute = 0;
 };
 
 inline void lt_mark(OptState* o, int what, hipStream_t st) {
@@ -386,8 +391,7 @@
             }
         }
         out->nch = nch;
-        out->ja_hi = 1;
-        for (int j = 0; j < NJ; ++j) if (csc_start[j + 1] > csc_start[j]) out->ja_hi = j + 1;
+        out->ja_hi = skin_ja_hi(csc_start.data(), NJ);
         HIP_TRY(out->csc_chunk.upload(cc.data(), cc.size()));
     }
     tr.mark("lists, vpack, chunk table");
diff --git a/include/fdcap.h b/include/fdcap.h
--- a/include/fdcap.h
+++ b/include/fdcap.h
@@ -203,6 +203,9 @@
 int fdcap_opt_nn_timing_read(fdcap_ctx* ctx, float* mean_ms, int32_t* launches);
 
 int fdcap_debug_nn_query_order(fdcap_ctx* ctx, int32_t mode, const int32_t* perm_h, int32_t n);
+int fdcap_debug_nn_records(fdcap_ctx* ctx, float* rec4_d, void* stream);
+int fdcap_debug_contact_diet(fdcap_ctx* ctx, int32_t* out4);
+int fdcap_debug_contact_perm(fdcap_ctx* ctx, int32_t* perm_h, int32_t n);
 
 int fdcap_debug_nn_query_sort(fdcap_ctx* ctx, const int32_t* pos_h, int32_t nq, int32_t groups, int32_t hdr_len, int32_t* hdr_io,
                               int32_t* perm_out, void* stream);
```

Measured after the change: 18720 frames/s (median of 6 runs). 1.01x the previous value.
